# JoeyYoung/adapcc

Measured on AMD Instinct MI355X. Metric: gpt2_ddp_tokens_per_sec, higher is better.
Workload: dtype bf16; 1 GPU; model=gpt2-small-124M, global_batch=128, seq_len=1024, parallelism=dp1, bucket_cap_mb=100, hipgraph=True, precision=bf16, transport=native

## Files before the change

adapcc_amd/models/gpt2.py:

```python

from __future__ import annotations

import math
from dataclasses import dataclass

import torch
import torch.nn as nn
import torch.nn.functional as F

from ..ops.fused import FusedLayerNorm


@dataclass
class GPT2Config:
    vocab_size: int = 50257
    n_positions: int = 1024
    n_embd: int = 768
    n_layer: int = 12
    n_head: int = 12
    dropout: float = 0.0
    resid_dropout: float = 0.0
    n_kv_head: int = None

    @classmethod
    def small(cls) -> "GPT2Config":
        return cls()

    @classmethod
    def tiny(cls) -> "GPT2Config":
        return cls(vocab_size=2048, n_positions=256, n_embd=128, n_layer=2,
                   n_head=4)

    @classmethod
    def medium(cls) -> "GPT2Config":
        return cls(n_embd=1024, n_layer=24, n_head=16)


class CausalSelfAttention(nn.Module):
    def __init__(self, cfg: GPT2Config):
        super().__init__()
        assert cfg.n_embd % cfg.n_head == 0
        self.n_head = cfg.n_head
        self.n_kv_head = (cfg.n_head if cfg.n_kv_head is None
                          else cfg.n_kv_head)
        assert self.n_kv_head >= 1 and cfg.n_head % self.n_kv_head == 0
        head_dim = cfg.n_embd // cfg.n_head
        self.c_attn = nn.Linear(
            cfg.n_embd, (cfg.n_head + 2 * self.n_kv_head) * head_dim)
        self.c_proj = nn.Linear(cfg.n_embd, cfg.n_embd)
        self.dropout = cfg.dropout

    def forward(self, x: torch.Tensor,
                cu_seqlens: torch.Tensor = None) -> torch.Tensor:
        from ..ops import attention

        p = self.dropout if self.training else 0.0
        if cu_seqlens is not None:
            qkv = self.c_attn(x)
            y = attention.flash_attention_qkv_varlen(
                qkv.view(qkv.shape[1], qkv.shape[2]), self.n_head,
                cu_seqlens, dropout_p=p, n_kv_head=self.n_kv_head)
            return self.c_proj(y.view(1, y.shape[0], y.shape[1]))
        return self.c_proj(attention.flash_attention_qkv(
            self.c_attn(x), self.n_head,
            dropout_p=self.dropout if self.training else 0.0,
            n_kv_head=self.n_kv_head,
        ))


class MLP(nn.Module):
    def __init__(self, cfg: GPT2Config):
        super().__init__()
        self.c_fc = nn.Linear(cfg.n_embd, 4 * cfg.n_embd)
        self.c_proj = nn.Linear(4 * cfg.n_embd, cfg.n_embd)

    def forward(self, x: torch.Tensor) -> torch.Tensor:
        from ..ops.fused import fused_gelu

        return self.c_proj(fused_gelu(self.c_fc(x)))


class Block(nn.Module):
    def __init__(self, cfg: GPT2Config):
        super().__init__()
        self.ln_1 = FusedLayerNorm(cfg.n_embd)
        self.attn = CausalSelfAttention(cfg)
        self.ln_2 = FusedLayerNorm(cfg.n_embd)
        self.mlp = MLP(cfg)

    def forward(self, x: torch.Tensor,
                cu_seqlens: torch.Tensor = None) -> torch.Tensor:
        if cu_seqlens is None:
            x = x + self.attn(self.ln_1(x))
        else:
            x = x + self.attn(self.ln_1(x), cu_seqlens)
        x = x + self.mlp(self.ln_2(x))
        return x

    def forward_resid_dropout(self, x: torch.Tensor, y: torch.Tensor,
                              next_ln: nn.LayerNorm, p: float, site: int,
                              cu_seqlens: torch.Tensor = None):
        from ..ops.fused import fused_dropout_add_layer_norm

        a = self.attn(y) if cu_seqlens is None else self.attn(y, cu_seqlens)
        x, y = fused_dropout_add_layer_norm(
            a, x, self.ln_2.weight, self.ln_2.bias, self.ln_2.eps,
            dropout_p=p, site=site)
        return fused_dropout_add_layer_norm(
            self.mlp(y), x, next_ln.weight, next_ln.bias, next_ln.eps,
            dropout_p=p, site=site + 1)


class GPT2(nn.Module):
    def __init__(self, cfg: GPT2Config):
        super().__init__()
        self.cfg = cfg
        self.wte = nn.Embedding(cfg.vocab_size, cfg.n_embd)
        self.wpe = nn.Embedding(cfg.n_positions, cfg.n_embd)
        self.drop = nn.Dropout(cfg.dropout)
        self.h = nn.ModuleList(Block(cfg) for _ in range(cfg.n_layer))
        self.ln_f = FusedLayerNorm(cfg.n_embd)
        self.lm_head = nn.Linear(cfg.n_embd, cfg.vocab_size, bias=False)
        self.lm_head.weight = self.wte.weight
        self.apply(self._init)
        for name, p in self.named_parameters():
            if name.endswith("c_proj.weight"):
                nn.init.normal_(p, mean=0.0,
                                std=0.02 / math.sqrt(2 * cfg.n_layer))

    @staticmethod
    def _init(m: nn.Module) -> None:
        if isinstance(m, nn.Linear):
            nn.init.normal_(m.weight, mean=0.0, std=0.02)
            if m.bias is not None:
                nn.init.zeros_(m.bias)
        elif isinstance(m, nn.Embedding):
            nn.init.normal_(m.weight, mean=0.0, std=0.02)

    def num_params(self, non_embedding: bool = True) -> int:
        n = sum(p.numel() for p in self.parameters())
        if non_embedding:
            n -= self.wpe.weight.numel()
        return n

    def _packed_positions(self, cu_seqlens: torch.Tensor,
                          total: int) -> torch.Tensor:
        rows = torch.arange(total, dtype=torch.int32,
                            device=cu_seqlens.device)
        ends = cu_seqlens[1:].contiguous()
        doc = torch.bucketize(rows, ends, right=True)
        doc = doc.clamp_(max=ends.numel() - 1)
        pos = rows - cu_seqlens[:-1][doc]
        return pos.clamp_(0, self.cfg.n_positions - 1).long()

    def forward(self, idx: torch.Tensor, targets: torch.Tensor = None,
                cu_seqlens: torch.Tensor = None):
        B, T = idx.shape
        if cu_seqlens is None:
            pos = torch.arange(T, device=idx.device)
            kw = {}
        else:
            if B != 1:
                raise ValueError("GPT2.forward: with cu_seqlens idx must be "
                                 f"[1, total], got {tuple(idx.shape)}")
            pos = self._packed_positions(cu_seqlens, T)
            kw = {"cu_seqlens": cu_seqlens}
        x = self.drop(self.wte(idx) + self.wpe(pos))
        if self.training and self.cfg.resid_dropout > 0.0:
            lns = [b.ln_1 for b in self.h[1:]] + [self.ln_f]
            y = self.h[0].ln_1(x)
            for i, block in enumerate(self.h):
                x, y = block.forward_resid_dropout(
                    x, y, lns[i], self.cfg.resid_dropout, site=2 * i, **kw)
            x = y
        else:
            for block in self.h:
                x = block(x, **kw)
            x = self.ln_f(x)
        logits = self.lm_head(x)
        loss = None
        if targets is not None:
            from ..ops.fused import fused_cross_entropy

            loss = fused_cross_entropy(
                logits.view(-1, logits.size(-1)), targets.view(-1)
            )
        return logits, loss
```

adapcc_amd/ops/build.py:

```python

from __future__ import annotations

import hashlib
import os
import subprocess
import sys
import sysconfig

PKG_DIR = os.path.dirname(os.path.dirname(os.path.abspath(__file__)))
CSRC = os.path.join(PKG_DIR, "ops", "csrc")
SOURCES = ["kernels.hip", "engine.hip", "plan.cpp", "lnorm.hip", "ce.hip",
           "attn.hip", "attn_probe.hip", "gelu.hip", "moe.hip",
           "bindings.hip"]
HEADERS = ["common.h", "engine.h", "plan.h", "attn_frag.h", "attn_drop.h"]
OUT_SO = os.path.join(PKG_DIR, "_core.so")
STAMP = os.path.join(PKG_DIR, "ops", ".build_stamp")

HIPCC = os.environ.get("ADAPCC_HIPCC", "/opt/rocm/bin/hipcc")
ARCH = os.environ.get("PYTORCH_ROCM_ARCH", "gfx950")


def _source_hash() -> str:
    h = hashlib.sha256()
    for name in SOURCES + HEADERS:
        with open(os.path.join(CSRC, name), "rb") as f:
            h.update(f.read())
    h.update(ARCH.encode())
    return h.hexdigest()


def needs_build() -> bool:
    if not os.path.exists(OUT_SO):
        return True
    if not os.path.exists(STAMP):
        return True
    with open(STAMP) as f:
        return f.read().strip() != _source_hash()


def build(verbose: bool = True, force: bool = False) -> str:
    if not force and not needs_build():
        return OUT_SO
    import pybind11

    py_inc = sysconfig.get_paths()["include"]
    cmd = [
        HIPCC,
        f"--offload-arch={ARCH}",
        "-O3",
        "-std=c++17",
        "-fPIC",
        "-shared",
        "-fvisibility=hidden",
        f"-I{CSRC}",
        f"-I{pybind11.get_include()}",
        f"-I{py_inc}",
    ]
    cmd += [os.path.join(CSRC, s) for s in SOURCES]
    cmd += ["-o", OUT_SO]
    if verbose:
        print("[adapcc_amd.build]", " ".join(cmd), file=sys.stderr)
    subprocess.run(cmd, check=True)
    with open(STAMP, "w") as f:
        f.write(_source_hash())
    return OUT_SO


if __name__ == "__main__":
    build(force="--force" in sys.argv)
```

adapcc_amd/ops/csrc/attn.hip:

```cpp

#include <algorithm>
#include <cmath>
#include <cstdint>
#include <stdexcept>
#include <string>
#include <type_traits>

#include "attn_drop.h"
#include "attn_frag.h"

namespace adapcc {

namespace {

constexpr int kQT = 128;
constexpr float kNegBig = -3.0e38f;
constexpr float kLog2e = 1.4426950408889634f;
constexpr float kLn2 = 0.6931471805599453f;

struct TStride {
  long sb, sh, ss;
};

template <typename T>
__device__ __forceinline__ T* plane(T* x, const TStride& s, int b, int h) {
  return x + (long)b * s.sb + (long)h * s.sh;
}

struct FaParams {
  const __bf16 *q, *k, *v;
  __bf16* o;
  float* lse;
  TStride qs, ks, vs, os;
  int H, S;
  float scale;
  const __bf16* dout;
  float* delta;
  __bf16 *dq, *dk, *dv;
  TStride dos_, dqs, dks, dvs;
  const long* seed;
  unsigned drop_thr;
  float drop_rp;
  const int4* tmap;
  int total;
  int G;
};

struct VarlenTile {
  int seq, tile, start, len;
};

__device__ __forceinline__ VarlenTile varlen_tile(const FaParams& p) {
  const int4 e = p.tmap[blockIdx.x];
  return {e.x, e.y, e.z, e.w};
}

template <bool kVarlen, typename T>
__device__ __forceinline__ T* seq_plane(T* x, const TStride& s, int b, int h,
                                        long row0) {
  if constexpr (kVarlen)
    return x + (long)h * s.sh + row0 * s.ss;
  else
    return plane(x, s, b, h);
}

template <bool kGqa>
__device__ __forceinline__ int kv_head(int h, int G) {
  if constexpr (kGqa)
    return h / G;
  else
    return h;
}

__device__ __forceinline__ bool varlen_idle(const VarlenTile& t) {
  return t.seq < 0 || (long)t.tile * kQT >= t.len;
}

template <bool kRagged>
__device__ __forceinline__ long ld_row(long row, int S) {
  return kRagged ? (long)min((int)row, S - 1) : row;
}
template <bool kRagged>
__device__ __forceinline__ int ld_row32(int row, int S) {
  return kRagged ? min(row, S - 1) : row;
}

template <bool kCausal, bool kRagged>
__device__ __forceinline__ int tile_count(int qt, int S) {
  if (kCausal && kRagged) return min((qt + 1) * (kQT / 64), (S + 63) / 64);
  return kCausal ? (qt + 1) * (kQT / 64) : (S + 63) / 64;
}

template <bool kCausal, bool kRagged>
__device__ __forceinline__ bool key_masked(int kglob, int qrow, int qlim,
                                           int S) {
  if (kCausal && kRagged) return kglob > qlim;
  return kCausal ? kglob > qrow : kglob >= S;
}

constexpr int kHalfImg = 4096;
constexpr int kImg = 2 * kHalfImg;

template <int kHD>
constexpr int kTileImg = (kHD / 64) * kImg;

template <int kHD>
__device__ __forceinline__ char* img(char* base, int buf) {
  return base + buf * kTileImg<kHD>;
}

template <int kHD>
__device__ __forceinline__ bf16x8 read_row_chunk(const char* im, int lane,
                                                 int c) {
  if constexpr (kHD == 64)
    return read_row_frag(im, lane, c);
  else
    return read_row_frag(im + (c >> 2) * kImg, lane, c & 3);
}

template <int kHD>
__device__ __forceinline__ bf16x8 read_tr_blk(const char* im, int lane,
                                              int kb, int db) {
  if constexpr (kHD == 64)
    return read_tr_frag(im, lane, kb, db);
  else
    return read_tr_frag(im + (db >> 1) * kImg, lane, kb, db & 1);
}

struct RowPair {
  uint4 a, b;
};

__device__ __forceinline__ RowPair ld_pair(const __bf16* g, long ss, long r0,
                                           long r1, int scol) {
  return {*reinterpret_cast<const uint4*>(g + r0 * ss + scol),
          *reinterpret_cast<const uint4*>(g + r1 * ss + scol)};
}

__device__ __forceinline__ void st_pair(char* im, int srow, int scol,
                                        const RowPair& x) {
  *reinterpret_cast<uint4*>(im + row_img_byte(srow, scol)) = x.a;
  *reinterpret_cast<uint4*>(im + kHalfImg + row_img_byte(srow, scol)) = x.b;
}

template <int kHD>
struct RowTile {
  RowPair blk[kHD / 64];
};

template <int kHD>
__device__ __forceinline__ RowTile<kHD> ld_tile(const __bf16* g, long ss,
                                                long r0, long r1, int scol) {
  RowTile<kHD> x;
  x.blk[0] = ld_pair(g, ss, r0, r1, scol);
  if constexpr (kHD == 128) x.blk[1] = ld_pair(g + 64, ss, r0, r1, scol);
  return x;
}

template <int kHD>
__device__ __forceinline__ void st_tile(char* im, int srow, int scol,
                                        const RowTile<kHD>& x) {
  st_pair(im, srow, scol, x.blk[0]);
  if constexpr (kHD == 128) st_pair(im + kImg, srow, scol, x.blk[1]);
}

constexpr int kSideDelta = 128;

struct SideVal {
  float lse2, delta;
};

__device__ __forceinline__ SideVal ld_side(const float* lseg,
                                           const float* deltag, int row) {
  return {lseg[row] * kLog2e, deltag[row]};
}

__device__ __forceinline__ float* side_buf(float* side, int buf) {
  return side + (buf ? 64 : 0);
}

__device__ __forceinline__ void st_side(float* side, int buf, unsigned i,
                                        const SideVal& x) {
  side[(buf ? 64 : 0) + i] = x.lse2;
  (side + kSideDelta)[(buf ? 64 : 0) + i] = x.delta;
}

template <bool kDrop>
constexpr int kPartBytes = kDrop ? 2 * 64 * 4 : 0;

__device__ __forceinline__ unsigned* part_buf(unsigned* part, int buf) {
  return part + (buf ? 64 : 0);
}

__device__ __forceinline__ void store4_bf16(__bf16* dst, float a, float b,
                                            float c, float d) {
  unsigned lo, hi;
  asm("v_cvt_pk_bf16_f32 %0, %2, %3\n\t"
      "v_cvt_pk_bf16_f32 %1, %4, %5"
      : "=&v"(lo), "=&v"(hi)
      : "v"(a), "v"(b), "v"(c), "v"(d));
  uint2 st = {lo, hi};
  *reinterpret_cast<uint2*>(dst) = st;
}

__device__ __forceinline__ float p_elem(float s, float c1, float off) {
  return __builtin_amdgcn_exp2f(__builtin_fmaf(s, c1, -off));
}

__device__ __forceinline__ float ds_elem(float pe, float dp, float delta,
                                         float scale) {
  return pe * (dp - delta) * scale;
}

template <int kHD, bool kCausal, bool kRagged, bool kDrop,
          bool kVarlen = false, bool kGqa = false>
__global__ __launch_bounds__(256, kHD == 64 ? 3 : 2) void fa_fwd_kernel(
    FaParams p) {
  static_assert(kHD == 64 || kHD == 128, "head_dim 64 or 128");
  static_assert(kVarlen ? kRagged : !(kCausal && kRagged),
                "fixed-length causal needs S % 128 == 0; varlen is ragged");
  constexpr int kNC = kHD / 16;
  constexpr int kNB = kHD / 32;
  __shared__ __attribute__((aligned(16))) char
      smem[4 * kTileImg<kHD> + kPartBytes<kDrop>];
  char* const kimg = smem;
  char* const vimg = smem + 2 * kTileImg<kHD>;
  [[maybe_unused]] unsigned* const kpart =
      reinterpret_cast<unsigned*>(smem + 4 * kTileImg<kHD>);

  const int lane = threadIdx.x & 63;
  const int wave = threadIdx.x >> 6;
  const int hi = lane >> 5;
  int qt = blockIdx.x, bh = blockIdx.y, b, h, S = p.S;
  long row0 = 0;
  if constexpr (kVarlen) {
    const VarlenTile vt = varlen_tile(p);
    if (varlen_idle(vt)) return;
    qt = vt.tile;
    b = 0;
    h = blockIdx.y;
    bh = vt.seq * p.H + h;
    S = vt.len;
    row0 = vt.start;
  } else {
    b = bh / p.H;
    h = bh % p.H;
  }

  const __bf16* qg = seq_plane<kVarlen>(p.q, p.qs, b, h, row0);
  const int hk = kv_head<kGqa>(h, p.G);
  const __bf16* kg = seq_plane<kVarlen>(p.k, p.ks, b, hk, row0);
  const __bf16* vg = seq_plane<kVarlen>(p.v, p.vs, b, hk, row0);
  __bf16* og = seq_plane<kVarlen>(p.o, p.os, b, h, row0);
  float* lseg =
      p.lse + (kVarlen ? (long)h * p.total + row0 : (long)bh * S);

  const int qb = qt * kQT + wave * 32;
  const int qrow = qb + (lane & 31);
  const long qld = ld_row<kRagged>((long)qrow, S);
  [[maybe_unused]] const int qlim = min(qrow, S - 1);

  bf16x8 qf[kNC];
#pragma unroll
  for (int c = 0; c < kNC; ++c)
    qf[c] = *reinterpret_cast<const bf16x8*>(
        qg + qld * p.qs.ss + c * 16 + hi * 8);

  f32x16 acc0 = {}, acc1 = {};
  [[maybe_unused]] f32x16 acc2 = {}, acc3 = {};
  float m = kNegBig, ssum = 0.f;
  const float c1 = p.scale * kLog2e;
  float mc = m * c1;
  const float thr = 8.0f / p.scale;

  const int srow = threadIdx.x >> 3;
  const int scol = (threadIdx.x & 7) * 8;
  const int n64 = tile_count<kCausal, kRagged>(qt, S);

  [[maybe_unused]] unsigned dqa = 0, seed_hi = 0;
  if constexpr (kDrop) {
    const unsigned long sd = (unsigned long)*p.seed;
    dqa = drop_q_part((unsigned)sd, bh, qrow);
    seed_hi = (unsigned)(sd >> 32);
  }

  {
    const long r0 = ld_row<kRagged>((long)srow, S);
    const long r1 = ld_row<kRagged>((long)(srow + 32), S);
    st_tile<kHD>(img<kHD>(kimg, 0), srow, scol,
                 ld_tile<kHD>(kg, p.ks.ss, r0, r1, scol));
    st_tile<kHD>(img<kHD>(vimg, 0), srow, scol,
                 ld_tile<kHD>(vg, p.vs.ss, r0, r1, scol));
    if constexpr (kDrop)
      if (threadIdx.x < 64)
        kpart[threadIdx.x] = drop_k_part(seed_hi, bh, threadIdx.x);
  }
  __syncthreads();

  int cur = 0;
  for (int t = 0; t < n64; ++t) {
    RowTile<kHD> nk, nv;
    const bool pref = t + 1 < n64;
    if (pref) {
      const long kb = (long)(t + 1) * 64 + srow;
      const long kb0 = ld_row<kRagged>(kb, S);
      const long kb1 = ld_row<kRagged>(kb + 32, S);
      nk = ld_tile<kHD>(kg, p.ks.ss, kb0, kb1, scol);
      nv = ld_tile<kHD>(vg, p.vs.ss, kb0, kb1, scol);
      if constexpr (kDrop)
        if (threadIdx.x < 64)
          part_buf(kpart, cur ^ 1)[threadIdx.x] =
              drop_k_part(seed_hi, bh, (t + 1) * 64 + threadIdx.x);
    }

#pragma unroll
    for (int half = 0; half < 2; ++half) {
      const int kbase = t * 64 + half * 32;
      if (kCausal) {
        if (kbase > qb + 31) break;
      }
      if (kRagged) {
        if (kbase >= S || qb >= S) break;
      }
      const char* ki = img<kHD>(kimg, cur) + half * kHalfImg;
      const char* vi = img<kHD>(vimg, cur) + half * kHalfImg;

      f32x16 s = {};
      __builtin_amdgcn_s_setprio(1);
#pragma unroll
      for (int c = 0; c < kNC; ++c)
        s = mfma(read_row_chunk<kHD>(ki, lane, c), qf[c], s);
      __builtin_amdgcn_s_setprio(0);

      float pv[16];
      float tmax = kNegBig;
      if ((kCausal && kbase + 31 > qb) || (kRagged && kbase + 31 >= S)) {
#pragma unroll
        for (int r = 0; r < 16; ++r) {
          const int kglob = kbase + crow(r, hi);
          pv[r] = key_masked<kCausal, kRagged>(kglob, qrow, qlim, S)
                      ? kNegBig
                      : s[r];
          tmax = fmaxf(tmax, pv[r]);
        }
      } else {
#pragma unroll
        for (int r = 0; r < 16; ++r) {
          pv[r] = s[r];
          tmax = fmaxf(tmax, pv[r]);
        }
      }
      tmax = fmaxf(tmax, __shfl_xor(tmax, 32, 64));
      if (!__all(tmax <= m + thr)) {
        const float mnew = fmaxf(m, tmax);
        const float alpha = __builtin_amdgcn_exp2f((m - mnew) * c1);
        m = mnew;
        mc = m * c1;
        ssum *= alpha;
#pragma unroll
        for (int r = 0; r < 16; ++r) {
          acc0[r] *= alpha;
          acc1[r] *= alpha;
          if constexpr (kNB == 4) {
            acc2[r] *= alpha;
            acc3[r] *= alpha;
          }
        }
      }

      float psum = 0.f;
#pragma unroll
      for (int r = 0; r < 16; ++r) {
        pv[r] = p_elem(pv[r], c1, mc);
        psum += pv[r];
      }
      ssum += psum;

      if constexpr (kDrop) {
        const unsigned* kp = part_buf(kpart, cur) + half * 32;
#pragma unroll
        for (int r = 0; r < 16; ++r)
          if (!drop_keep_parts(dqa, kp[crow(r, hi)], p.drop_thr))
            pv[r] = 0.f;
      }

      const bf16x8 p0 = pack_frag(&pv[0]);
      const bf16x8 p1 = pack_frag(&pv[8]);

      __builtin_amdgcn_s_setprio(1);
      acc0 = mfma(read_tr_blk<kHD>(vi, lane, 0, 0), p0, acc0);
      acc0 = mfma(read_tr_blk<kHD>(vi, lane, 1, 0), p1, acc0);
      acc1 = mfma(read_tr_blk<kHD>(vi, lane, 0, 1), p0, acc1);
      acc1 = mfma(read_tr_blk<kHD>(vi, lane, 1, 1), p1, acc1);
      if constexpr (kNB == 4) {
        acc2 = mfma(read_tr_blk<kHD>(vi, lane, 0, 2), p0, acc2);
        acc2 = mfma(read_tr_blk<kHD>(vi, lane, 1, 2), p1, acc2);
        acc3 = mfma(read_tr_blk<kHD>(vi, lane, 0, 3), p0, acc3);
        acc3 = mfma(read_tr_blk<kHD>(vi, lane, 1, 3), p1, acc3);
      }
      __builtin_amdgcn_s_setprio(0);
    }

    if (pref) {
      st_tile<kHD>(img<kHD>(kimg, cur ^ 1), srow, scol, nk);
      st_tile<kHD>(img<kHD>(vimg, cur ^ 1), srow, scol, nv);
    }
    __syncthreads();
    cur ^= 1;
  }

  const float stot = ssum + __shfl_xor(ssum, 32, 64);
  float inv = 1.f / stot;
  if constexpr (kDrop) inv = p.drop_rp / stot;
  if (kRagged && qrow >= S) return;
  if ((lane >> 5) == 0)
    lseg[qrow] = p.scale * m + __builtin_amdgcn_logf(stot) * kLn2;

  __bf16* orow = og + (long)qrow * p.os.ss;
#pragma unroll
  for (int db = 0; db < kNB; ++db) {
    const f32x16& a = db == 3 ? acc3 : db == 2 ? acc2 : db ? acc1 : acc0;
#pragma unroll
    for (int mq = 0; mq < 4; ++mq)
      store4_bf16(orow + db * 32 + 8 * mq + 4 * hi, a[4 * mq] * inv,
                  a[4 * mq + 1] * inv, a[4 * mq + 2] * inv,
                  a[4 * mq + 3] * inv);
  }
}

__device__ __forceinline__ float dot8_tree(bf16x8 a, bf16x8 b) {
  union {
    bf16x8 f;
    unsigned u[4];
  } x, y;
  x.f = a;
  y.f = b;
  float pr[4];
#pragma unroll
  for (int i = 0; i < 4; ++i) {
    const float ev = __builtin_fmaf(__uint_as_float(x.u[i] << 16),
                                    __uint_as_float(y.u[i] << 16), 0.f);
    pr[i] = __builtin_fmaf(__uint_as_float(x.u[i] & 0xffff0000u),
                           __uint_as_float(y.u[i] & 0xffff0000u), ev);
  }
  return (pr[0] + pr[1]) + (pr[2] + pr[3]);
}

template <int kHD, bool kCausal, bool kRagged, bool kDrop,
          bool kVarlen = false, bool kGqa = false>
__global__ __launch_bounds__(256, kHD == 64 ? 3 : 2) void fa_bwd_dq_kernel(
    FaParams p) {
  static_assert(kHD == 64 || kHD == 128, "head_dim 64 or 128");
  static_assert(kVarlen ? kRagged : !(kCausal && kRagged),
                "fixed-length causal needs S % 128 == 0; varlen is ragged");
  constexpr int kNC = kHD / 16;
  constexpr int kNB = kHD / 32;
  __shared__ __attribute__((aligned(16))) char
      smem[4 * kTileImg<kHD> + kPartBytes<kDrop>];
  char* const kimg = smem;
  char* const vimg = smem + 2 * kTileImg<kHD>;
  [[maybe_unused]] unsigned* const kpart =
      reinterpret_cast<unsigned*>(smem + 4 * kTileImg<kHD>);

  const int lane = threadIdx.x & 63;
  const int wave = threadIdx.x >> 6;
  const int hi = lane >> 5;
  int qt = blockIdx.x, bh = blockIdx.y, b, h, S = p.S;
  long row0 = 0;
  if constexpr (kVarlen) {
    const VarlenTile vt = varlen_tile(p);
    if (varlen_idle(vt)) return;
    qt = vt.tile;
    b = 0;
    h = blockIdx.y;
    bh = vt.seq * p.H + h;
    S = vt.len;
    row0 = vt.start;
  } else {
    b = bh / p.H;
    h = bh % p.H;
  }

  const __bf16* qg = seq_plane<kVarlen>(p.q, p.qs, b, h, row0);
  const int hk = kv_head<kGqa>(h, p.G);
  const __bf16* kg = seq_plane<kVarlen>(p.k, p.ks, b, hk, row0);
  const __bf16* vg = seq_plane<kVarlen>(p.v, p.vs, b, hk, row0);
  const __bf16* dog = seq_plane<kVarlen>(p.dout, p.dos_, b, h, row0);
  const __bf16* og = seq_plane<kVarlen>(p.o, p.os, b, h, row0);
  __bf16* dqg = seq_plane<kVarlen>(p.dq, p.dqs, b, h, row0);
  const long lrow0 = kVarlen ? (long)h * p.total + row0 : (long)bh * S;

  const int qb = qt * kQT + wave * 32;
  const int qrow = qb + (lane & 31);
  const long qld = ld_row32<kRagged>(qrow, S);
  [[maybe_unused]] const int qlim = min(qrow, S - 1);

  bf16x8 qf[kNC], dof[kNC];
  float n16[kNC];
#pragma unroll
  for (int c = 0; c < kNC; ++c) {
    dof[c] = *reinterpret_cast<const bf16x8*>(
        dog + qld * p.dos_.ss + c * 16 + hi * 8);
    const float n8 = dot8_tree(
        dof[c], *reinterpret_cast<const bf16x8*>(
                    og + qld * p.os.ss + c * 16 + hi * 8));
    n16[c] = n8 + __shfl_xor(n8, 32, 64);
  }
#pragma unroll
  for (int c = 0; c < kNC; ++c)
    qf[c] = *reinterpret_cast<const bf16x8*>(
        qg + qld * p.qs.ss + c * 16 + hi * 8);
  const float lse2 = p.lse[lrow0 + qld] * kLog2e;
  float dvq = (n16[0] + n16[1]) + (n16[2] + n16[3]);
  if constexpr (kHD == 128)
    dvq = dvq + ((n16[4] + n16[5]) + (n16[6] + n16[7]));
  if (hi == 0 && (!kRagged || qrow < S))
    p.delta[lrow0 + qrow] = dvq;
  const float c1 = p.scale * kLog2e;

  f32x16 dacc0 = {}, dacc1 = {};
  [[maybe_unused]] f32x16 dacc2 = {}, dacc3 = {};

  const int srow = threadIdx.x >> 3;
  const int scol = (threadIdx.x & 7) * 8;
  const int n64 = tile_count<kCausal, kRagged>(qt, S);

  [[maybe_unused]] unsigned dqa = 0, seed_hi = 0;
  if constexpr (kDrop) {
    const unsigned long sd = (unsigned long)*p.seed;
    dqa = drop_q_part((unsigned)sd, bh, qrow);
    seed_hi = (unsigned)(sd >> 32);
  }
  {
    const long r0 = ld_row32<kRagged>(srow, S);
    const long r1 = ld_row32<kRagged>(srow + 32, S);
    st_tile<kHD>(img<kHD>(kimg, 0), srow, scol,
                 ld_tile<kHD>(kg, p.ks.ss, r0, r1, scol));
    st_tile<kHD>(img<kHD>(vimg, 0), srow, scol,
                 ld_tile<kHD>(vg, p.vs.ss, r0, r1, scol));
    if constexpr (kDrop)
      if (threadIdx.x < 64)
        kpart[threadIdx.x] = drop_k_part(seed_hi, bh, threadIdx.x);
  }
  __syncthreads();

  int cur = 0;
  for (int t = 0; t < n64; ++t) {
    RowTile<kHD> nk, nv;
    const bool pref = t + 1 < n64;
    if (pref) {
      const long kb0 = ld_row32<kRagged>((t + 1) * 64 + srow, S);
      const long kb1 = ld_row32<kRagged>((t + 1) * 64 + srow + 32, S);
      nk = ld_tile<kHD>(kg, p.ks.ss, kb0, kb1, scol);
      nv = ld_tile<kHD>(vg, p.vs.ss, kb0, kb1, scol);
      if constexpr (kDrop)
        if (threadIdx.x < 64)
          part_buf(kpart, cur ^ 1)[threadIdx.x] =
              drop_k_part(seed_hi, bh, (t + 1) * 64 + threadIdx.x);
    }

#pragma unroll
    for (int half = 0; half < 2; ++half) {
      const int kbase = t * 64 + half * 32;
      if (kCausal) {
        if (kbase > qb + 31) break;
      }
      if (kRagged) {
        if (kbase >= S || qb >= S) break;
      }
      const char* ki = img<kHD>(kimg, cur) + half * kHalfImg;
      const char* vi = img<kHD>(vimg, cur) + half * kHalfImg;

      f32x16 s = {}, dp = {};
      __builtin_amdgcn_s_setprio(1);
#pragma unroll
      for (int c = 0; c < kNC; ++c) {
        s = mfma(read_row_chunk<kHD>(ki, lane, c), qf[c], s);
        dp = mfma(read_row_chunk<kHD>(vi, lane, c), dof[c], dp);
      }
      __builtin_amdgcn_s_setprio(0);

      float ds[16];
      [[maybe_unused]] const unsigned* kp =
          part_buf(kpart, cur) + half * 32;
      auto dpk = [&](int r) {
        if constexpr (kDrop)
          return drop_keep_parts(dqa, kp[crow(r, hi)], p.drop_thr)
                     ? dp[r] * p.drop_rp
                     : 0.f;
        else
          return dp[r];
      };
      if (kDrop) {
        const int lim = kCausal ? (kRagged ? qlim : qrow)
                        : kRagged ? S - 1
                                  : 0x7fffffff;
#pragma unroll
        for (int r = 0; r < 16; ++r) {
          const int kglob = kbase + crow(r, hi);
          const float pe = kglob > lim ? 0.f : p_elem(s[r], c1, lse2);
          ds[r] = ds_elem(pe, dpk(r), dvq, p.scale);
        }
      } else if ((kCausal && kbase + 31 > qb) ||
                 (kRagged && kbase + 31 >= S)) {
#pragma unroll
        for (int r = 0; r < 16; ++r) {
          const int kglob = kbase + crow(r, hi);
          const float pe = key_masked<kCausal, kRagged>(kglob, qrow, qlim, S)
                               ? 0.f
                               : p_elem(s[r], c1, lse2);
          ds[r] = ds_elem(pe, dpk(r), dvq, p.scale);
        }
      } else {
#pragma unroll
        for (int r = 0; r < 16; ++r)
          ds[r] = ds_elem(p_elem(s[r], c1, lse2), dpk(r), dvq, p.scale);
      }
      const bf16x8 d0 = pack_frag(&ds[0]);
      const bf16x8 d1 = pack_frag(&ds[8]);
      __builtin_amdgcn_s_setprio(1);
      dacc0 = mfma(read_tr_blk<kHD>(ki, lane, 0, 0), d0, dacc0);
      dacc0 = mfma(read_tr_blk<kHD>(ki, lane, 1, 0), d1, dacc0);
      dacc1 = mfma(read_tr_blk<kHD>(ki, lane, 0, 1), d0, dacc1);
      dacc1 = mfma(read_tr_blk<kHD>(ki, lane, 1, 1), d1, dacc1);
      if constexpr (kNB == 4) {
        dacc2 = mfma(read_tr_blk<kHD>(ki, lane, 0, 2), d0, dacc2);
        dacc2 = mfma(read_tr_blk<kHD>(ki, lane, 1, 2), d1, dacc2);
        dacc3 = mfma(read_tr_blk<kHD>(ki, lane, 0, 3), d0, dacc3);
        dacc3 = mfma(read_tr_blk<kHD>(ki, lane, 1, 3), d1, dacc3);
      }
      __builtin_amdgcn_s_setprio(0);
    }

    if (pref) {
      st_tile<kHD>(img<kHD>(kimg, cur ^ 1), srow, scol, nk);
      st_tile<kHD>(img<kHD>(vimg, cur ^ 1), srow, scol, nv);
    }
    __syncthreads();
    cur ^= 1;
  }

  if (kRagged && qrow >= S) return;
  __bf16* drow = dqg + (long)qrow * p.dqs.ss;
#pragma unroll
  for (int db = 0; db < kNB; ++db) {
    const f32x16& a = db == 3 ? dacc3 : db == 2 ? dacc2 : db ? dacc1 : dacc0;
#pragma unroll
    for (int mq = 0; mq < 4; ++mq)
      store4_bf16(drow + db * 32 + 8 * mq + 4 * hi, a[4 * mq], a[4 * mq + 1],
                  a[4 * mq + 2], a[4 * mq + 3]);
  }
}

template <int kHD, bool kCausal, bool kRagged, bool kDrop,
          bool kVarlen = false, bool kGqa = false>
__global__ __launch_bounds__(256, kHD == 64 ? 2 : 1) void fa_bwd_dkv_kernel(
    FaParams p) {
  static_assert(kHD == 64 || kHD == 128, "head_dim 64 or 128");
  static_assert(kVarlen ? kRagged : !(kCausal && kRagged),
                "fixed-length causal needs S % 128 == 0; varlen is ragged");
  constexpr int kNC = kHD / 16;
  constexpr int kNB = kHD / 32;
  __shared__ __attribute__((aligned(16))) char
      smem[4 * kTileImg<kHD> + 1024 + kPartBytes<kDrop>];
  char* const qimg = smem;
  char* const doimg = smem + 2 * kTileImg<kHD>;
  float* const side =
      reinterpret_cast<float*>(smem + 4 * kTileImg<kHD>);
  [[maybe_unused]] unsigned* const qpart =
      reinterpret_cast<unsigned*>(smem + 4 * kTileImg<kHD> + 1024);

  const int lane = threadIdx.x & 63;
  const int wave = threadIdx.x >> 6;
  const int hi = lane >> 5;
  int kt = blockIdx.x, bh = blockIdx.y, b, h, S = p.S;
  int hk;
  long row0 = 0;
  if constexpr (kVarlen) {
    const VarlenTile vt = varlen_tile(p);
    if (varlen_idle(vt)) return;
    kt = vt.tile;
    b = 0;
    hk = blockIdx.y;
    h = kGqa ? hk * p.G : hk;
    bh = vt.seq * p.H + h;
    S = vt.len;
    row0 = vt.start;
  } else if constexpr (kGqa) {
    const int Hk = p.H / p.G;
    b = bh / Hk;
    hk = bh % Hk;
    h = hk * p.G;
    bh = b * p.H + h;
  } else {
    b = bh / p.H;
    h = bh % p.H;
    hk = h;
  }

  const __bf16* qg = seq_plane<kVarlen>(p.q, p.qs, b, h, row0);
  const __bf16* kg = seq_plane<kVarlen>(p.k, p.ks, b, hk, row0);
  const __bf16* vg = seq_plane<kVarlen>(p.v, p.vs, b, hk, row0);
  const __bf16* dog = seq_plane<kVarlen>(p.dout, p.dos_, b, h, row0);
  __bf16* dkg = seq_plane<kVarlen>(p.dk, p.dks, b, hk, row0);
  __bf16* dvg = seq_plane<kVarlen>(p.dv, p.dvs, b, hk, row0);
  const long lrow0 = kVarlen ? (long)h * p.total + row0 : (long)bh * S;
  const float* lseg = p.lse + lrow0;
  const float* deltag = p.delta + lrow0;

  const int kbb = kt * kQT + wave * 32;
  const int krow = kbb + (lane & 31);
  const long kld = ld_row32<kRagged>(krow, S);

  bf16x8 kf[kNC], vf[kNC];
#pragma unroll
  for (int c = 0; c < kNC; ++c) {
    kf[c] = *reinterpret_cast<const bf16x8*>(
        kg + kld * p.ks.ss + c * 16 + hi * 8);
    vf[c] = *reinterpret_cast<const bf16x8*>(
        vg + kld * p.vs.ss + c * 16 + hi * 8);
  }

  const float c1 = p.scale * kLog2e;
  f32x16 dvacc0 = {}, dvacc1 = {}, dkacc0 = {}, dkacc1 = {};
  [[maybe_unused]] f32x16 dvacc2 = {}, dvacc3 = {}, dkacc2 = {}, dkacc3 = {};

  const int srow = threadIdx.x >> 3;
  const int scol = (threadIdx.x & 7) * 8;
  const int t0 = kCausal ? (kVarlen ? kt * (kQT / 64) : kt) : 0;
  const int n64 = (S + 63) / 64;

  [[maybe_unused]] unsigned dkb = 0, seed_lo = 0;
  [[maybe_unused]] unsigned seed_hi = 0;
  [[maybe_unused]] int bhc = bh;
  if constexpr (kDrop) {
    const unsigned long sd = (unsigned long)*p.seed;
    seed_lo = (unsigned)sd;
    dkb = drop_k_part((unsigned)(sd >> 32), bh, krow);
    if constexpr (kGqa) seed_hi = (unsigned)(sd >> 32);
  }
  [[maybe_unused]] int stage_left = 0, walk_left = 0;
  if constexpr (kGqa) stage_left = walk_left = p.G - 1;

  {
    const int qb0 = t0 * 64;
    const long r0 = ld_row32<kRagged>(qb0 + srow, S);
    const long r1 = ld_row32<kRagged>(qb0 + srow + 32, S);
    st_tile<kHD>(img<kHD>(qimg, 0), srow, scol,
                 ld_tile<kHD>(qg, p.qs.ss, r0, r1, scol));
    st_tile<kHD>(img<kHD>(doimg, 0), srow, scol,
                 ld_tile<kHD>(dog, p.dos_.ss, r0, r1, scol));
    if (threadIdx.x < 64) {
      const int rq = ld_row32<kRagged>(qb0 + (int)threadIdx.x, S);
      st_side(side, 0, threadIdx.x, ld_side(lseg, deltag, rq));
      if constexpr (kDrop)
        qpart[threadIdx.x] = drop_q_part(seed_lo, bh, qb0 + threadIdx.x);
    }
  }
  __syncthreads();

  int cur = 0;
  for (int t = t0; t < n64; ++t) {
    RowTile<kHD> nq, nd;
    SideVal ns = {0.f, 0.f};
    bool pref = t + 1 < n64;
    int tn = t + 1;
    if constexpr (kGqa) {
      if (!pref && stage_left > 0) {
        --stage_left;
        pref = true;
        tn = t0;
        qg += p.qs.sh;
        dog += p.dos_.sh;
        lseg += kVarlen ? p.total : S;
        deltag += kVarlen ? p.total : S;
        ++bh;
      }
    }
    if (pref) {
      const int qb1 = tn * 64;
      const long r0 = ld_row32<kRagged>(qb1 + srow, S);
      const long r1 = ld_row32<kRagged>(qb1 + srow + 32, S);
      nq = ld_tile<kHD>(qg, p.qs.ss, r0, r1, scol);
      nd = ld_tile<kHD>(dog, p.dos_.ss, r0, r1, scol);
      if (threadIdx.x < 64) {
        const int rq = ld_row32<kRagged>(qb1 + (int)threadIdx.x, S);
        ns = ld_side(lseg, deltag, rq);
        if constexpr (kDrop)
          part_buf(qpart, cur ^ 1)[threadIdx.x] =
              drop_q_part(seed_lo, bh, qb1 + threadIdx.x);
      }
    }

#pragma unroll
    for (int half = 0; half < 2; ++half) {
      const int qbase = t * 64 + half * 32;
      if (kCausal) {
        if (qbase + 31 < kbb) continue;
      }
      if (kRagged) {
        if (qbase >= S || kbb >= S) break;
      }
      const char* qi = img<kHD>(qimg, cur) + half * kHalfImg;
      const char* di = img<kHD>(doimg, cur) + half * kHalfImg;
      const float* lsec = side_buf(side, cur) + half * 32;
      const float* dc = lsec + kSideDelta;

      f32x16 sacc = {}, dp = {};
      __builtin_amdgcn_s_setprio(1);
#pragma unroll
      for (int c = 0; c < kNC; ++c) {
        sacc = mfma(read_row_chunk<kHD>(qi, lane, c), kf[c], sacc);
        dp = mfma(read_row_chunk<kHD>(di, lane, c), vf[c], dp);
      }
      __builtin_amdgcn_s_setprio(0);

      float pv[16], ds[16];
      [[maybe_unused]] bool keep[16];
      if constexpr (kDrop) {
        const unsigned* qp = part_buf(qpart, cur) + half * 32;
#pragma unroll
        for (int r = 0; r < 16; ++r) {
          keep[r] = drop_keep_parts(qp[crow(r, hi)], dkb, p.drop_thr);
          dp[r] = keep[r] ? dp[r] * p.drop_rp : 0.f;
        }
      }
      if ((kCausal && qbase < kbb + 31) || (kRagged && qbase + 31 >= S)) {
#pragma unroll
        for (int r = 0; r < 16; ++r) {
          const int qglob = qbase + crow(r, hi);
          pv[r] = ((kCausal && qglob < krow) || (kRagged && qglob >= S))
                      ? 0.f
                      : p_elem(sacc[r], c1, lsec[crow(r, hi)]);
          ds[r] = ds_elem(pv[r], dp[r], dc[crow(r, hi)], p.scale);
        }
      } else {
#pragma unroll
        for (int r = 0; r < 16; ++r) {
          pv[r] = p_elem(sacc[r], c1, lsec[crow(r, hi)]);
          ds[r] = ds_elem(pv[r], dp[r], dc[crow(r, hi)], p.scale);
        }
      }
      if constexpr (kDrop) {
#pragma unroll
        for (int r = 0; r < 16; ++r)
          if (!keep[r]) pv[r] = 0.f;
      }
      const bf16x8 p0 = pack_frag(&pv[0]);
      const bf16x8 p1 = pack_frag(&pv[8]);
      __builtin_amdgcn_s_setprio(1);
      dvacc0 = mfma(p0, read_tr_blk<kHD>(di, lane, 0, 0), dvacc0);
      dvacc0 = mfma(p1, read_tr_blk<kHD>(di, lane, 1, 0), dvacc0);
      dvacc1 = mfma(p0, read_tr_blk<kHD>(di, lane, 0, 1), dvacc1);
      dvacc1 = mfma(p1, read_tr_blk<kHD>(di, lane, 1, 1), dvacc1);
      if constexpr (kNB == 4) {
        dvacc2 = mfma(p0, read_tr_blk<kHD>(di, lane, 0, 2), dvacc2);
        dvacc2 = mfma(p1, read_tr_blk<kHD>(di, lane, 1, 2), dvacc2);
        dvacc3 = mfma(p0, read_tr_blk<kHD>(di, lane, 0, 3), dvacc3);
        dvacc3 = mfma(p1, read_tr_blk<kHD>(di, lane, 1, 3), dvacc3);
      }
      __builtin_amdgcn_s_setprio(0);
      const bf16x8 e0 = pack_frag(&ds[0]);
      const bf16x8 e1 = pack_frag(&ds[8]);
      __builtin_amdgcn_s_setprio(1);
      dkacc0 = mfma(e0, read_tr_blk<kHD>(qi, lane, 0, 0), dkacc0);
      dkacc0 = mfma(e1, read_tr_blk<kHD>(qi, lane, 1, 0), dkacc0);
      dkacc1 = mfma(e0, read_tr_blk<kHD>(qi, lane, 0, 1), dkacc1);
      dkacc1 = mfma(e1, read_tr_blk<kHD>(qi, lane, 1, 1), dkacc1);
      if constexpr (kNB == 4) {
        dkacc2 = mfma(e0, read_tr_blk<kHD>(qi, lane, 0, 2), dkacc2);
        dkacc2 = mfma(e1, read_tr_blk<kHD>(qi, lane, 1, 2), dkacc2);
        dkacc3 = mfma(e0, read_tr_blk<kHD>(qi, lane, 0, 3), dkacc3);
        dkacc3 = mfma(e1, read_tr_blk<kHD>(qi, lane, 1, 3), dkacc3);
      }
      __builtin_amdgcn_s_setprio(0);
    }

    if (pref) {
      st_tile<kHD>(img<kHD>(qimg, cur ^ 1), srow, scol, nq);
      st_tile<kHD>(img<kHD>(doimg, cur ^ 1), srow, scol, nd);
      if (threadIdx.x < 64) st_side(side, cur ^ 1, threadIdx.x, ns);
    }
    __syncthreads();
    cur ^= 1;
    if constexpr (kGqa) {
      if (t + 1 == n64 && walk_left > 0) {
        --walk_left;
        t = t0 - 1;
        if constexpr (kDrop) dkb = drop_k_part(seed_hi, ++bhc, krow);
      }
    }
  }

  __syncthreads();
  float* scratch = reinterpret_cast<float*>(smem) + wave * (32 * kHD);
#pragma unroll
  for (int t = 0; t < 2; ++t) {
    const f32x16& a0 = t ? dkacc0 : dvacc0;
    const f32x16& a1 = t ? dkacc1 : dvacc1;
    [[maybe_unused]] const f32x16& a2 = t ? dkacc2 : dvacc2;
    [[maybe_unused]] const f32x16& a3 = t ? dkacc3 : dvacc3;
    if (kDrop && t == 0) {
#pragma unroll
      for (int r = 0; r < 16; ++r) {
        scratch[crow(r, hi) * kHD + (lane & 31)] = a0[r] * p.drop_rp;
        scratch[crow(r, hi) * kHD + 32 + (lane & 31)] = a1[r] * p.drop_rp;
        if constexpr (kNB == 4) {
          scratch[crow(r, hi) * kHD + 64 + (lane & 31)] = a2[r] * p.drop_rp;
          scratch[crow(r, hi) * kHD + 96 + (lane & 31)] = a3[r] * p.drop_rp;
        }
      }
    } else {
#pragma unroll
      for (int r = 0; r < 16; ++r) {
        scratch[crow(r, hi) * kHD + (lane & 31)] = a0[r];
        scratch[crow(r, hi) * kHD + 32 + (lane & 31)] = a1[r];
        if constexpr (kNB == 4) {
          scratch[crow(r, hi) * kHD + 64 + (lane & 31)] = a2[r];
          scratch[crow(r, hi) * kHD + 96 + (lane & 31)] = a3[r];
        }
      }
    }
    __builtin_amdgcn_s_waitcnt(0);
    __bf16* outg = (t ? dkg : dvg);
    const TStride& os = t ? p.dks : p.dvs;
    const int row = lane >> 1;
    const int dhalf = (lane & 1) * (kHD / 2);
#pragma unroll
    for (int mq = 0; mq < kHD / 8; ++mq) {
      const float* src = scratch + row * kHD + dhalf + mq * 4;
      if (!kRagged || kbb + row < S)
        store4_bf16(outg + (long)(kbb + row) * os.ss + dhalf + mq * 4, src[0],
                    src[1], src[2], src[3]);
    }
    __syncthreads();
  }
}

__global__ __launch_bounds__(256) void fa_dropout_mask_kernel(
    uint8_t* out, const long* seed, int S, unsigned thr) {
  const long n = (long)S * S;
  const long i = (long)blockIdx.x * 256 + threadIdx.x;
  if (i >= n) return;
  const unsigned bh = blockIdx.y;
  out[bh * n + i] =
      drop_keep(*seed, bh, (unsigned)(i / S), (unsigned)(i % S), thr);
}

constexpr int kIntMin = -2147483647 - 1;

template <bool kMax>
__device__ __forceinline__ int plan_scan(int* buf, int x, int* all) {
  const int t = threadIdx.x;
  constexpr int kId = kMax ? kIntMin : 0;
  buf[t] = x;
  __syncthreads();
  for (int d = 1; d < 256; d <<= 1) {
    const int y = t >= d ? buf[t - d] : kId;
    __syncthreads();
    buf[t] = kMax ? max(buf[t], y) : buf[t] + y;
    __syncthreads();
  }
  const int excl = t ? buf[t - 1] : kId;
  *all = buf[255];
  __syncthreads();
  return excl;
}

__device__ __forceinline__ int clamp_row(int x, int total) {
  return min(max(x, 0), total);
}

__global__ __launch_bounds__(256) void fa_varlen_plan_kernel(
    const int* cu, int n_seqs, int total, int max_tiles, int4* tmap) {
  __shared__ int buf[256];
  const int t = threadIdx.x;
  const int per = (n_seqs + 255) / 256;
  const int i0 = min(t * per, n_seqs), i1 = min(i0 + per, n_seqs);

  int mx = kIntMin;
  for (int i = i0; i < i1; ++i) mx = max(mx, cu[i + 1]);
  int unused;
  const int m0 = max(cu[0], plan_scan<true>(buf, mx, &unused));

  int tiles = 0;
  for (int i = i0, m = m0; i < i1; ++i) {
    const int e = clamp_row(m, total);
    m = max(m, cu[i + 1]);
    tiles += (clamp_row(m, total) - e + kQT - 1) / kQT;
  }
  int n_tiles;
  int at = plan_scan<false>(buf, tiles, &n_tiles);

  for (int i = i0, m = m0; i < i1; ++i) {
    const int e = clamp_row(m, total);
    m = max(m, cu[i + 1]);
    const int len = clamp_row(m, total) - e;
    for (int j = 0; j * kQT < len; ++j, ++at)
      if (at < max_tiles) tmap[at] = make_int4(i, j, e, len);
  }
  for (int x = n_tiles + t; x < max_tiles; x += 256)
    tmap[x] = make_int4(-1, -1, -1, -1);
}

TStride stride_at(const long* s, int i) {
  return {s[3 * i], s[3 * i + 1], s[3 * i + 2]};
}

unsigned drop_threshold(double p) {
  const double t = std::nearbyint(p * 4294967296.0);
  return (unsigned)std::min(std::max(t, 1.0), 4294967295.0);
}

void check_drop(const char* name, double p, const long* seed) {
  if (!(p >= 0.0 && p < 1.0))
    throw std::runtime_error(std::string(name) + ": need 0 <= dropout_p < 1");
  if (p > 0.0 && seed == nullptr)
    throw std::runtime_error(std::string(name) +
                             ": dropout needs a device seed");
}

void set_drop(FaParams& p, double dropout_p, const long* seed) {
  p.seed = seed;
  p.drop_thr = drop_threshold(dropout_p);
  p.drop_rp = (float)(1.0 / (1.0 - dropout_p));
}

void check_len(const char* name, int S, bool causal) {
  if (S < 1) throw std::runtime_error(std::string(name) + ": S < 1");
  if (causal && S % kQT != 0)
    throw std::runtime_error(std::string(name) +
                             ": causal needs S % 128 == 0");
}

void check_varlen(const char* name, int total, int n_seqs, int H) {
  if (total < 1) throw std::runtime_error(std::string(name) + ": total < 1");
  if (n_seqs < 1)
    throw std::runtime_error(std::string(name) + ": n_seqs < 1");
  if (H < 1) throw std::runtime_error(std::string(name) + ": H < 1");
  if ((long)total / kQT + n_seqs > 0x7fffffffL - kQT || total > 0x7fffff00)
    throw std::runtime_error(std::string(name) + ": too many tiles");
}

int varlen_max_tiles(int total, int n_seqs) { return total / kQT + n_seqs; }

template <typename F>
void with_mode(bool causal, int S, bool drop, bool varlen, F&& f) {
  auto g = [&](auto d) {
    if (varlen) {
      if (causal)
        f(std::true_type{}, std::true_type{}, d, std::true_type{});
      else
        f(std::false_type{}, std::true_type{}, d, std::true_type{});
    } else if (causal) {
      f(std::true_type{}, std::false_type{}, d, std::false_type{});
    } else if (S % kQT == 0) {
      f(std::false_type{}, std::false_type{}, d, std::false_type{});
    } else {
      f(std::false_type{}, std::true_type{}, d, std::false_type{});
    }
  };
  if (drop)
    g(std::true_type{});
  else
    g(std::false_type{});
}

FaParams fwd_params(const char* name, const void* q, const void* k,
                    const void* v, void* o, float* lse, int H, int n_kv_head,
                    int S, const long* strides, float scale) {
  const int Hk = n_kv_head == 0 ? H : n_kv_head;
  if (H < 1 || Hk < 1 || H % Hk != 0)
    throw std::runtime_error(std::string(name) + ": need n_kv_head >= 1 that "
                             "divides H, got H " + std::to_string(H) +
                             ", n_kv_head " + std::to_string(n_kv_head));
  FaParams p = {};
  p.G = H / Hk;
  p.q = (const __bf16*)q;
  p.k = (const __bf16*)k;
  p.v = (const __bf16*)v;
  p.o = (__bf16*)o;
  p.lse = lse;
  p.qs = stride_at(strides, 0);
  p.ks = stride_at(strides, 1);
  p.vs = stride_at(strides, 2);
  p.os = stride_at(strides, 3);
  p.H = H;
  p.S = S;
  p.scale = scale;
  return p;
}

void bwd_params(FaParams& p, const void* do_, float* delta, void* dq,
                void* dk, void* dv, const long* strides) {
  p.dout = (const __bf16*)do_;
  p.delta = delta;
  p.dq = (__bf16*)dq;
  p.dk = (__bf16*)dk;
  p.dv = (__bf16*)dv;
  p.dos_ = stride_at(strides, 4);
  p.dqs = stride_at(strides, 5);
  p.dks = stride_at(strides, 6);
  p.dvs = stride_at(strides, 7);
}

void set_varlen(FaParams& p, const int* tmap, int total) {
  if (tmap == nullptr) throw std::runtime_error("fa_varlen: no tile map");
  p.tmap = reinterpret_cast<const int4*>(tmap);
  p.total = total;
}

template <typename F>
void with_head_dim(const char* name, int head_dim, F&& f) {
  if (head_dim == 64)
    f(std::integral_constant<int, 64>{});
  else if (head_dim == 128)
    f(std::integral_constant<int, 128>{});
  else
    throw std::runtime_error(std::string(name) +
                             ": head_dim must be 64 or 128, got " +
                             std::to_string(head_dim));
}

template <typename F>
void with_gqa(int G, F&& f) {
  if (G > 1)
    f(std::true_type{});
  else
    f(std::false_type{});
}

void launch_fwd(const FaParams& p, dim3 grid, int head_dim, bool causal,
                bool drop, bool varlen, hipStream_t stream) {
  with_head_dim("fa_forward", head_dim, [&](auto hd) {
    with_mode(causal, p.S, drop, varlen, [&](auto c, auto r, auto d, auto vl) {
      with_gqa(p.G, [&](auto gq) {
        constexpr int kHD = decltype(hd)::value;
        constexpr bool kC = decltype(c)::value, kR = decltype(r)::value,
                       kD = decltype(d)::value, kV = decltype(vl)::value,
                       kG = decltype(gq)::value;
        hipLaunchKernelGGL((fa_fwd_kernel<kHD, kC, kR, kD, kV, kG>), grid,
                           dim3(256), 0, stream, p);
      });
    });
  });
}

void launch_bwd(const FaParams& p, dim3 grid, int head_dim, bool causal,
                bool drop, bool varlen, hipStream_t stream) {
  const dim3 kv_grid(grid.x, grid.y / p.G);
  with_head_dim("fa_backward", head_dim, [&](auto hd) {
    with_mode(causal, p.S, drop, varlen, [&](auto c, auto r, auto d, auto vl) {
      with_gqa(p.G, [&](auto gq) {
        constexpr int kHD = decltype(hd)::value;
        constexpr bool kC = decltype(c)::value, kR = decltype(r)::value,
                       kD = decltype(d)::value, kV = decltype(vl)::value,
                       kG = decltype(gq)::value;
        hipLaunchKernelGGL((fa_bwd_dq_kernel<kHD, kC, kR, kD, kV, kG>), grid,
                           dim3(256), 0, stream, p);
        hipLaunchKernelGGL((fa_bwd_dkv_kernel<kHD, kC, kR, kD, kV, kG>),
                           kv_grid, dim3(256), 0, stream, p);
      });
    });
  });
}

}

unsigned fa_drop_threshold(double p) { return drop_threshold(p); }

void fa_forward(const void* q, const void* k, const void* v, void* o,
                float* lse, int B, int H, int S, const long* strides,
                float scale, hipStream_t stream, bool causal,
                double dropout_p, const long* seed, int head_dim,
                int n_kv_head) {
  check_len("fa_forward", S, causal);
  check_drop("fa_forward", dropout_p, seed);
  FaParams p = fwd_params("fa_forward", q, k, v, o, lse, H, n_kv_head, S,
                          strides, scale);
  set_drop(p, dropout_p, seed);
  const dim3 grid((S + kQT - 1) / kQT, B * H);
  launch_fwd(p, grid, head_dim, causal, dropout_p > 0.0, false, stream);
}

void fa_backward(const void* q, const void* k, const void* v, const void* o,
                 const void* do_, const float* lse, float* delta, void* dq,
                 void* dk, void* dv, int B, int H, int S, const long* strides,
                 float scale, hipStream_t stream, bool causal,
                 double dropout_p, const long* seed, int head_dim,
                 int n_kv_head) {
  check_len("fa_backward", S, causal);
  check_drop("fa_backward", dropout_p, seed);
  FaParams p = fwd_params("fa_backward", q, k, v, const_cast<void*>(o),
                          const_cast<float*>(lse), H, n_kv_head, S, strides,
                          scale);
  set_drop(p, dropout_p, seed);
  bwd_params(p, do_, delta, dq, dk, dv, strides);
  const dim3 grid((S + kQT - 1) / kQT, B * H);
  launch_bwd(p, grid, head_dim, causal, dropout_p > 0.0, false, stream);
}

void fa_varlen_plan(const int* cu_seqlens, int n_seqs, int total, int* tmap,
                    hipStream_t stream) {
  check_varlen("fa_varlen_plan", total, n_seqs, 1);
  if (cu_seqlens == nullptr || tmap == nullptr)
    throw std::runtime_error("fa_varlen_plan: null pointer");
  hipLaunchKernelGGL(fa_varlen_plan_kernel, dim3(1), dim3(256), 0, stream,
                     cu_seqlens, n_seqs, total,
                     varlen_max_tiles(total, n_seqs),
                     reinterpret_cast<int4*>(tmap));
}

void fa_varlen_forward(const void* q, const void* k, const void* v, void* o,
                       float* lse, const int* tmap, int total, int n_seqs,
                       int H, const long* strides, float scale,
                       hipStream_t stream, bool causal, double dropout_p,
                       const long* seed, int head_dim, int n_kv_head) {
  check_varlen("fa_varlen_forward", total, n_seqs, H);
  check_drop("fa_varlen_forward", dropout_p, seed);
  FaParams p = fwd_params("fa_varlen_forward", q, k, v, o, lse, H, n_kv_head,
                          0, strides, scale);
  set_drop(p, dropout_p, seed);
  set_varlen(p, tmap, total);
  const dim3 grid(varlen_max_tiles(total, n_seqs), H);
  launch_fwd(p, grid, head_dim, causal, dropout_p > 0.0, true, stream);
}

void fa_varlen_backward(const void* q, const void* k, const void* v,
                        const void* o, const void* do_, const float* lse,
                        float* delta, void* dq, void* dk, void* dv,
                        const int* tmap, int total, int n_seqs, int H,
                        const long* strides, float scale, hipStream_t stream,
                        bool causal, double dropout_p, const long* seed,
                        int head_dim, int n_kv_head) {
  check_varlen("fa_varlen_backward", total, n_seqs, H);
  check_drop("fa_varlen_backward", dropout_p, seed);
  FaParams p = fwd_params("fa_varlen_backward", q, k, v,
                          const_cast<void*>(o), const_cast<float*>(lse), H,
                          n_kv_head, 0, strides, scale);
  set_drop(p, dropout_p, seed);
  set_varlen(p, tmap, total);
  bwd_params(p, do_, delta, dq, dk, dv, strides);
  const dim3 grid(varlen_max_tiles(total, n_seqs), H);
  launch_bwd(p, grid, head_dim, causal, dropout_p > 0.0, true, stream);
}

void fa_dropout_mask(uint8_t* out, const long* seed, int B, int H, int S,
                     double dropout_p, hipStream_t stream) {
  if (S < 1 || B < 1 || H < 1)
    throw std::runtime_error("fa_dropout_mask: empty shape");
  if (seed == nullptr)
    throw std::runtime_error("fa_dropout_mask: needs a device seed");
  check_drop("fa_dropout_mask", dropout_p, seed);
  const long n = (long)S * S;
  const dim3 grid((unsigned)((n + 255) / 256), B * H);
  hipLaunchKernelGGL(fa_dropout_mask_kernel, grid, dim3(256), 0, stream, out,
                     seed, S, drop_threshold(dropout_p));
}

}
```

adapcc_amd/ops/csrc/bindings.hip:

```cpp

#include <pybind11/pybind11.h>
#include <pybind11/stl.h>

#include "common.h"
#include "engine.h"
#include "plan.h"

namespace py = pybind11;
using adapcc::Engine;

static py::dict plan_to_dict(const adapcc::PlanData& p) {
  py::list cs, rs, bs;
  for (const auto& u : p.cunits) {
    py::dict d;
    d["tree"] = u.tree; d["chunk"] = u.chunk;
    d["offset"] = u.offset_elems; d["count"] = u.count_elems;
    d["flag_space"] = (int)u.flag_space;
    py::list nl;
    for (int i = 0; i < u.nnotify; ++i) nl.append(u.notify_rank[i]);
    d["notify_to"] = nl;
    cs.append(d);
  }
  for (const auto& u : p.runits) {
    py::dict d;
    d["tree"] = u.tree; d["chunk"] = u.chunk;
    d["offset"] = u.offset_elems; d["count"] = u.count_elems;
    py::list srcs;
    for (int s = 0; s < u.nsrc; ++s)
      srcs.append(py::make_tuple(u.src_rank[s], (int)u.src_kind[s]));
    d["srcs"] = srcs;
    d["include_self"] = (bool)u.include_self;
    d["notify"] = (bool)u.notify_parent; d["consumer"] = u.parent_rank;
    d["is_root"] = (bool)u.is_root;
    py::list kids;
    for (int c = 0; c < u.nchildren; ++c) kids.append(u.child_rank[c]);
    d["publish_to"] = kids;
    rs.append(d);
  }
  for (const auto& u : p.bunits) {
    py::dict d;
    d["tree"] = u.tree; d["chunk"] = u.chunk;
    d["src_offset"] = u.src_offset_elems; d["dst_offset"] = u.dst_offset_elems;
    d["count"] = u.count_elems;
    d["parent"] = u.parent_rank; d["parent_kind"] = (int)u.parent_kind;
    d["forward"] = (bool)u.forward;
    py::list kids;
    for (int c = 0; c < u.nchildren; ++c) kids.append(u.child_rank[c]);
    d["publish_to"] = kids;
    bs.append(d);
  }
  py::dict out;
  out["copy"] = cs;
  out["reduce"] = rs;
  out["bcast"] = bs;
  out["chunk_elems"] = p.chunk_elems;
  return out;
}

namespace adapcc {
void launch_local_reduce(Dtype dt, void* dst, const void* const* srcs_dev,
                         int nsrc, long count, RedOp op, float scale,
                         hipStream_t stream);
bool ln_supported_api(long cols, int dtype);
void ln_forward(int dtype, const void* x, const void* w, const void* b,
                void* y, float* mean, float* rstd, long rows, long cols,
                float eps, hipStream_t stream);
void ln_backward(int dtype, const void* dy, const void* x, const void* w,
                 const float* mean, const float* rstd, void* dx,
                 float* ws_gamma, float* ws_beta, long rows, long cols,
                 int nblocks, hipStream_t stream);
void ln_dropadd_forward(int dtype, const void* h, const void* res,
                        const void* w, const void* b, void* x_new, void* y,
                        float* mean, float* rstd, long rows, long cols,
                        float eps, double dropout_p, const long* seed,
                        unsigned site, hipStream_t stream);
void ln_dropadd_backward(int dtype, const void* dy, const void* dx_new,
                         const void* x_new, const void* w, const float* mean,
                         const float* rstd, void* dres, void* dh,
                         float* ws_gamma, float* ws_beta, long rows,
                         long cols, int nblocks, double dropout_p,
                         const long* seed, unsigned site,
                         hipStream_t stream);
void ce_forward(int dtype, const void* logits, const void* targets,
                float* loss, float* lse, long rows, long cols,
                long ignore_index, hipStream_t stream);
void ce_backward(int dtype, const void* logits, const void* targets,
                 const float* lse, const float* gscale, void* dlogits,
                 long rows, long cols, long ignore_index, hipStream_t stream);
void fa_forward(const void* q, const void* k, const void* v, void* o,
                float* lse, int B, int H, int S, const long* strides,
                float scale, hipStream_t stream, bool causal,
                double dropout_p, const long* seed, int head_dim,
                int n_kv_head);
void fa_backward(const void* q, const void* k, const void* v, const void* o,
                 const void* do_, const float* lse, float* delta, void* dq,
                 void* dk, void* dv, int B, int H, int S, const long* strides,
                 float scale, hipStream_t stream, bool causal,
                 double dropout_p, const long* seed, int head_dim,
                 int n_kv_head);
void fa_dropout_mask(uint8_t* out, const long* seed, int B, int H, int S,
                     double dropout_p, hipStream_t stream);
void fa_varlen_plan(const int* cu_seqlens, int n_seqs, int total, int* tmap,
                    hipStream_t stream);
void fa_varlen_forward(const void* q, const void* k, const void* v, void* o,
                       float* lse, const int* tmap, int total, int n_seqs,
                       int H, const long* strides, float scale,
                       hipStream_t stream, bool causal, double dropout_p,
                       const long* seed, int head_dim, int n_kv_head);
void fa_varlen_backward(const void* q, const void* k, const void* v,
                        const void* o, const void* do_, const float* lse,
                        float* delta, void* dq, void* dk, void* dv,
                        const int* tmap, int total, int n_seqs, int H,
                        const long* strides, float scale, hipStream_t stream,
                        bool causal, double dropout_p, const long* seed,
                        int head_dim, int n_kv_head);
void mfma_probe(const void* a, const void* b, float* c, hipStream_t stream);
void gelu_forward(int dtype, const void* x, void* y, long n,
                  hipStream_t stream);
void gelu_backward(int dtype, const void* x, const void* dy, void* dx, long n,
                   hipStream_t stream);
void moe_route(int dtype, const void* logits, float* gate_p, int* expert,
               int* slot, int* src, int* counts, int* offs, int* totals,
               long ntok, long E, long cap, hipStream_t stream);
void moe_route_bwd(int dtype, const void* logits, const float* gate_p,
                   const int* expert, const int* slot, const float* dgate,
                   void* dlogits, long ntok, long E, hipStream_t stream);
void moe_route_topk(int dtype, const void* logits, int k, int normalize,
                    float* gate, float* pmax, int* expert, int* slot,
                    int* src, int* src_choice, int* load, float* aux,
                    int* counts, int* offs, int* totals, float* psum,
                    long ntok, long E, long cap, hipStream_t stream);
void moe_route_topk_bwd(int dtype, const void* logits, int k, int normalize,
                        const float* pmax, const float* gate,
                        const int* expert, const int* slot,
                        const float* dgate, const int* load,
                        const float* daux, void* dlogits, long ntok, long E,
                        hipStream_t stream);
void moe_gather(int dtype, const void* in, long in_rows, const int* map,
                const float* scale, int scale_by_src, const int* choice,
                int nchoice, void* out, long rows, long d,
                hipStream_t stream);
void moe_gather2(int dtype, const void* in, long in_rows, const int* map,
                 const float* scale, void* out, long rows, long d,
                 hipStream_t stream);
void moe_rowdot(int dtype, const void* a, const void* b, long b_rows,
                const int* map, float* out, long rows, long d, int a_shift,
                hipStream_t stream);
void tr_probe(float* out, int kb, int db, hipStream_t stream);
void pack_probe(float* out, hipStream_t stream);
}

PYBIND11_MODULE(_core, m) {
  m.doc() = "adapcc_amd native engine (MI355X / gfx950)";

  m.def("local_reduce",
        [](uintptr_t dst, const std::vector<uintptr_t>& srcs, long count,
           int dtype, int op, float scale, uintptr_t stream) {
          if (srcs.empty()) throw std::runtime_error("no sources");
          void** d_srcs = nullptr;
          hipError_t e = hipMalloc(&d_srcs, srcs.size() * sizeof(void*));
          if (e != hipSuccess) throw std::runtime_error(hipGetErrorString(e));
          e = hipMemcpy(d_srcs, srcs.data(), srcs.size() * sizeof(void*),
                        hipMemcpyHostToDevice);
          if (e != hipSuccess) throw std::runtime_error(hipGetErrorString(e));
          adapcc::launch_local_reduce(
              (adapcc::Dtype)dtype, reinterpret_cast<void*>(dst),
              (const void* const*)d_srcs, (int)srcs.size(), count,
              (adapcc::RedOp)op, scale, reinterpret_cast<hipStream_t>(stream));
          e = hipGetLastError();
          if (e != hipSuccess) throw std::runtime_error(hipGetErrorString(e));
          e = hipStreamSynchronize(reinterpret_cast<hipStream_t>(stream));
          (void)hipFree(d_srcs);
          if (e != hipSuccess) throw std::runtime_error(hipGetErrorString(e));
        },
        py::arg("dst"), py::arg("srcs"), py::arg("count"), py::arg("dtype"),
        py::arg("op"), py::arg("scale") = 1.0f, py::arg("stream") = 0);

  m.def("ln_supported", &adapcc::ln_supported_api, py::arg("cols"),
        py::arg("dtype"));
  m.def("ln_fwd",
        [](int dtype, uintptr_t x, uintptr_t w, uintptr_t b, uintptr_t y,
           uintptr_t mean, uintptr_t rstd, long rows, long cols, float eps,
           uintptr_t stream) {
          adapcc::ln_forward(dtype, (const void*)x, (const void*)w,
                             (const void*)b, (void*)y, (float*)mean,
                             (float*)rstd, rows, cols, eps,
                             reinterpret_cast<hipStream_t>(stream));
          hipError_t e = hipGetLastError();
          if (e != hipSuccess) throw std::runtime_error(hipGetErrorString(e));
        });
  m.def("ln_bwd",
        [](int dtype, uintptr_t dy, uintptr_t x, uintptr_t w, uintptr_t mean,
           uintptr_t rstd, uintptr_t dx, uintptr_t wsg, uintptr_t wsb,
           long rows, long cols, int nblocks, uintptr_t stream) {
          adapcc::ln_backward(dtype, (const void*)dy, (const void*)x,
                              (const void*)w, (const float*)mean,
                              (const float*)rstd, (void*)dx, (float*)wsg,
                              (float*)wsb, rows, cols, nblocks,
                              reinterpret_cast<hipStream_t>(stream));
          hipError_t e = hipGetLastError();
          if (e != hipSuccess) throw std::runtime_error(hipGetErrorString(e));
        });
  m.def("ln_dropadd_fwd",
        [](int dtype, uintptr_t h, uintptr_t res, uintptr_t w, uintptr_t b,
           uintptr_t x_new, uintptr_t y, uintptr_t mean, uintptr_t rstd,
           long rows, long cols, float eps, uintptr_t stream,
           double dropout_p, uintptr_t seed, unsigned site) {
          adapcc::ln_dropadd_forward(
              dtype, (const void*)h, (const void*)res, (const void*)w,
              (const void*)b, (void*)x_new, (void*)y, (float*)mean,
              (float*)rstd, rows, cols, eps, dropout_p, (const long*)seed,
              site, reinterpret_cast<hipStream_t>(stream));
          hipError_t e = hipGetLastError();
          if (e != hipSuccess) throw std::runtime_error(hipGetErrorString(e));
        },
        py::arg("dtype"), py::arg("h"), py::arg("res"), py::arg("w"),
        py::arg("b"), py::arg("x_new"), py::arg("y"), py::arg("mean"),
        py::arg("rstd"), py::arg("rows"), py::arg("cols"), py::arg("eps"),
        py::arg("stream"), py::arg("dropout_p") = 0.0, py::arg("seed") = 0,
        py::arg("site") = 0);
  m.def("ln_dropadd_bwd",
        [](int dtype, uintptr_t dy, uintptr_t dx_new, uintptr_t x_new,
           uintptr_t w, uintptr_t mean, uintptr_t rstd, uintptr_t dres,
           uintptr_t dh, uintptr_t wsg, uintptr_t wsb, long rows, long cols,
           int nblocks, uintptr_t stream, double dropout_p, uintptr_t seed,
           unsigned site) {
          adapcc::ln_dropadd_backward(
              dtype, (const void*)dy, (const void*)dx_new,
              (const void*)x_new, (const void*)w, (const float*)mean,
              (const float*)rstd, (void*)dres, (void*)dh, (float*)wsg,
              (float*)wsb, rows, cols, nblocks, dropout_p, (const long*)seed,
              site, reinterpret_cast<hipStream_t>(stream));
          hipError_t e = hipGetLastError();
          if (e != hipSuccess) throw std::runtime_error(hipGetErrorString(e));
        },
        py::arg("dtype"), py::arg("dy"), py::arg("dx_new"), py::arg("x_new"),
        py::arg("w"), py::arg("mean"), py::arg("rstd"), py::arg("dres"),
        py::arg("dh"), py::arg("wsg"), py::arg("wsb"), py::arg("rows"),
        py::arg("cols"), py::arg("nblocks"), py::arg("stream"),
        py::arg("dropout_p") = 0.0, py::arg("seed") = 0,
        py::arg("site") = 0);

  m.def("ce_fwd",
        [](int dtype, uintptr_t logits, uintptr_t targets, uintptr_t loss,
           uintptr_t lse, long rows, long cols, long ignore_index,
           uintptr_t stream) {
          adapcc::ce_forward(dtype, (const void*)logits,
                             (const void*)targets, (float*)loss, (float*)lse,
                             rows, cols, ignore_index,
                             reinterpret_cast<hipStream_t>(stream));
          hipError_t e = hipGetLastError();
          if (e != hipSuccess) throw std::runtime_error(hipGetErrorString(e));
        });
  m.def("ce_bwd",
        [](int dtype, uintptr_t logits, uintptr_t targets, uintptr_t lse,
           uintptr_t gscale, uintptr_t dlogits, long rows, long cols,
           long ignore_index, uintptr_t stream) {
          adapcc::ce_backward(dtype, (const void*)logits,
                              (const void*)targets, (const float*)lse,
                              (const float*)gscale, (void*)dlogits, rows,
                              cols, ignore_index,
                              reinterpret_cast<hipStream_t>(stream));
          hipError_t e = hipGetLastError();
          if (e != hipSuccess) throw std::runtime_error(hipGetErrorString(e));
        });

  m.def("fa_fwd",
        [](uintptr_t q, uintptr_t k, uintptr_t v, uintptr_t o, uintptr_t lse,
           int B, int H, int S, const std::vector<long>& strides, float scale,
           uintptr_t stream, bool causal, double dropout_p, uintptr_t seed,
           int head_dim, int n_kv_head) {
          if (strides.size() != 12)
            throw std::runtime_error("fa_fwd: need 12 strides");
          adapcc::fa_forward((const void*)q, (const void*)k, (const void*)v,
                             (void*)o, (float*)lse, B, H, S, strides.data(),
                             scale, reinterpret_cast<hipStream_t>(stream),
                             causal, dropout_p, (const long*)seed, head_dim,
                             n_kv_head);
          hipError_t e = hipGetLastError();
          if (e != hipSuccess) throw std::runtime_error(hipGetErrorString(e));
        },
        py::arg("q"), py::arg("k"), py::arg("v"), py::arg("o"),
        py::arg("lse"), py::arg("B"), py::arg("H"), py::arg("S"),
        py::arg("strides"), py::arg("scale"), py::arg("stream"),
        py::arg("causal") = true, py::arg("dropout_p") = 0.0,
        py::arg("seed") = 0, py::arg("head_dim") = 64,
        py::arg("n_kv_head") = 0);
  m.def("fa_bwd",
        [](uintptr_t q, uintptr_t k, uintptr_t v, uintptr_t o, uintptr_t dout,
           uintptr_t lse, uintptr_t delta, uintptr_t dq, uintptr_t dk,
           uintptr_t dv, int B, int H, int S, const std::vector<long>& strides,
           float scale, uintptr_t stream, bool causal, double dropout_p,
           uintptr_t seed, int head_dim, int n_kv_head) {
          if (strides.size() != 24)
            throw std::runtime_error("fa_bwd: need 24 strides");
          adapcc::fa_backward((const void*)q, (const void*)k, (const void*)v,
                              (const void*)o, (const void*)dout,
                              (const float*)lse, (float*)delta, (void*)dq,
                              (void*)dk, (void*)dv, B, H, S, strides.data(),
                              scale, reinterpret_cast<hipStream_t>(stream),
                              causal, dropout_p, (const long*)seed, head_dim,
                              n_kv_head);
          hipError_t e = hipGetLastError();
          if (e != hipSuccess) throw std::runtime_error(hipGetErrorString(e));
        },
        py::arg("q"), py::arg("k"), py::arg("v"), py::arg("o"),
        py::arg("dout"), py::arg("lse"), py::arg("delta"), py::arg("dq"),
        py::arg("dk"), py::arg("dv"), py::arg("B"), py::arg("H"),
        py::arg("S"), py::arg("strides"), py::arg("scale"),
        py::arg("stream"), py::arg("causal") = true,
        py::arg("dropout_p") = 0.0, py::arg("seed") = 0,
        py::arg("head_dim") = 64, py::arg("n_kv_head") = 0);
  m.def("fa_dropout_mask",
        [](uintptr_t out, uintptr_t seed, int B, int H, int S,
           double dropout_p, uintptr_t stream) {
          adapcc::fa_dropout_mask((uint8_t*)out, (const long*)seed, B, H, S,
                                  dropout_p,
                                  reinterpret_cast<hipStream_t>(stream));
          hipError_t e = hipGetLastError();
          if (e != hipSuccess) throw std::runtime_error(hipGetErrorString(e));
        },
        py::arg("out"), py::arg("seed"), py::arg("B"), py::arg("H"),
        py::arg("S"), py::arg("dropout_p"), py::arg("stream"));
  m.def("fa_varlen_plan",
        [](uintptr_t cu_seqlens, int n_seqs, int total, uintptr_t tmap,
           uintptr_t stream) {
          adapcc::fa_varlen_plan((const int*)cu_seqlens, n_seqs, total,
                                 (int*)tmap,
                                 reinterpret_cast<hipStream_t>(stream));
          hipError_t e = hipGetLastError();
          if (e != hipSuccess) throw std::runtime_error(hipGetErrorString(e));
        },
        py::arg("cu_seqlens"), py::arg("n_seqs"), py::arg("total"),
        py::arg("tmap"), py::arg("stream"));
  m.def("fa_varlen_fwd",
        [](uintptr_t q, uintptr_t k, uintptr_t v, uintptr_t o, uintptr_t lse,
           uintptr_t tmap, int total, int n_seqs, int H,
           const std::vector<long>& strides, float scale, uintptr_t stream,
           bool causal, double dropout_p, uintptr_t seed, int head_dim,
           int n_kv_head) {
          if (strides.size() != 12)
            throw std::runtime_error("fa_varlen_fwd: need 12 strides");
          adapcc::fa_varlen_forward(
              (const void*)q, (const void*)k, (const void*)v, (void*)o,
              (float*)lse, (const int*)tmap, total, n_seqs, H, strides.data(),
              scale, reinterpret_cast<hipStream_t>(stream), causal, dropout_p,
              (const long*)seed, head_dim, n_kv_head);
          hipError_t e = hipGetLastError();
          if (e != hipSuccess) throw std::runtime_error(hipGetErrorString(e));
        },
        py::arg("q"), py::arg("k"), py::arg("v"), py::arg("o"),
        py::arg("lse"), py::arg("tmap"), py::arg("total"), py::arg("n_seqs"),
        py::arg("H"), py::arg("strides"), py::arg("scale"), py::arg("stream"),
        py::arg("causal") = true, py::arg("dropout_p") = 0.0,
        py::arg("seed") = 0, py::arg("head_dim") = 64,
        py::arg("n_kv_head") = 0);
  m.def("fa_varlen_bwd",
        [](uintptr_t q, uintptr_t k, uintptr_t v, uintptr_t o, uintptr_t dout,
           uintptr_t lse, uintptr_t delta, uintptr_t dq, uintptr_t dk,
           uintptr_t dv, uintptr_t tmap, int total, int n_seqs, int H,
           const std::vector<long>& strides, float scale, uintptr_t stream,
           bool causal, double dropout_p, uintptr_t seed, int head_dim,
           int n_kv_head) {
          if (strides.size() != 24)
            throw std::runtime_error("fa_varlen_bwd: need 24 strides");
          adapcc::fa_varlen_backward(
              (const void*)q, (const void*)k, (const void*)v, (const void*)o,
              (const void*)dout, (const float*)lse, (float*)delta, (void*)dq,
              (void*)dk, (void*)dv, (const int*)tmap, total, n_seqs, H,
              strides.data(), scale, reinterpret_cast<hipStream_t>(stream),
              causal, dropout_p, (const long*)seed, head_dim, n_kv_head);
          hipError_t e = hipGetLastError();
          if (e != hipSuccess) throw std::runtime_error(hipGetErrorString(e));
        },
        py::arg("q"), py::arg("k"), py::arg("v"), py::arg("o"),
        py::arg("dout"), py::arg("lse"), py::arg("delta"), py::arg("dq"),
        py::arg("dk"), py::arg("dv"), py::arg("tmap"), py::arg("total"),
        py::arg("n_seqs"), py::arg("H"), py::arg("strides"),
        py::arg("scale"), py::arg("stream"), py::arg("causal") = true,
        py::arg("dropout_p") = 0.0, py::arg("seed") = 0,
        py::arg("head_dim") = 64, py::arg("n_kv_head") = 0);
  m.def("mfma_probe",
        [](uintptr_t a, uintptr_t b, uintptr_t c, uintptr_t stream) {
          adapcc::mfma_probe((const void*)a, (const void*)b, (float*)c,
                             reinterpret_cast<hipStream_t>(stream));
          hipError_t e = hipGetLastError();
          if (e != hipSuccess) throw std::runtime_error(hipGetErrorString(e));
        });

  m.def("gelu_fwd",
        [](int dtype, uintptr_t x, uintptr_t y, long n, uintptr_t stream) {
          adapcc::gelu_forward(dtype, (const void*)x, (void*)y, n,
                               reinterpret_cast<hipStream_t>(stream));
          hipError_t e = hipGetLastError();
          if (e != hipSuccess) throw std::runtime_error(hipGetErrorString(e));
        });
  m.def("gelu_bwd",
        [](int dtype, uintptr_t x, uintptr_t dy, uintptr_t dx, long n,
           uintptr_t stream) {
          adapcc::gelu_backward(dtype, (const void*)x, (const void*)dy,
                                (void*)dx, n,
                                reinterpret_cast<hipStream_t>(stream));
          hipError_t e = hipGetLastError();
          if (e != hipSuccess) throw std::runtime_error(hipGetErrorString(e));
        });

  m.def("moe_route",
        [](int dtype, uintptr_t logits, uintptr_t gate_p, uintptr_t expert,
           uintptr_t slot, uintptr_t src, uintptr_t counts, uintptr_t offs,
           uintptr_t totals, long ntok, long E, long cap, uintptr_t stream) {
          adapcc::moe_route(dtype, (const void*)logits, (float*)gate_p,
                            (int*)expert, (int*)slot, (int*)src, (int*)counts,
                            (int*)offs, (int*)totals, ntok, E, cap,
                            reinterpret_cast<hipStream_t>(stream));
          hipError_t e = hipGetLastError();
          if (e != hipSuccess) throw std::runtime_error(hipGetErrorString(e));
        });
  m.def("moe_route_bwd",
        [](int dtype, uintptr_t logits, uintptr_t gate_p, uintptr_t expert,
           uintptr_t slot, uintptr_t dgate, uintptr_t dlogits, long ntok,
           long E, uintptr_t stream) {
          adapcc::moe_route_bwd(dtype, (const void*)logits,
                                (const float*)gate_p, (const int*)expert,
                                (const int*)slot, (const float*)dgate,
                                (void*)dlogits, ntok, E,
                                reinterpret_cast<hipStream_t>(stream));
          hipError_t e = hipGetLastError();
          if (e != hipSuccess) throw std::runtime_error(hipGetErrorString(e));
        });
  m.def("moe_route_topk",
        [](int dtype, uintptr_t logits, int k, bool normalize, uintptr_t gate,
           uintptr_t pmax, uintptr_t expert, uintptr_t slot, uintptr_t src,
           uintptr_t src_choice, uintptr_t load, uintptr_t aux,
           uintptr_t counts, uintptr_t offs, uintptr_t totals, uintptr_t psum,
           long ntok, long E, long cap, uintptr_t stream) {
          adapcc::moe_route_topk(
              dtype, (const void*)logits, k, normalize ? 1 : 0, (float*)gate,
              (float*)pmax, (int*)expert, (int*)slot, (int*)src,
              (int*)src_choice, (int*)load, (float*)aux, (int*)counts,
              (int*)offs, (int*)totals, (float*)psum, ntok, E, cap,
              reinterpret_cast<hipStream_t>(stream));
          hipError_t e = hipGetLastError();
          if (e != hipSuccess) throw std::runtime_error(hipGetErrorString(e));
        });
  m.def("moe_route_topk_bwd",
        [](int dtype, uintptr_t logits, int k, bool normalize, uintptr_t pmax,
           uintptr_t gate, uintptr_t expert, uintptr_t slot, uintptr_t dgate,
           uintptr_t load, uintptr_t daux, uintptr_t dlogits, long ntok,
           long E, uintptr_t stream) {
          adapcc::moe_route_topk_bwd(
              dtype, (const void*)logits, k, normalize ? 1 : 0,
              (const float*)pmax, (const float*)gate, (const int*)expert,
              (const int*)slot, (const float*)dgate, (const int*)load,
              (const float*)daux, (void*)dlogits, ntok, E,
              reinterpret_cast<hipStream_t>(stream));
          hipError_t e = hipGetLastError();
          if (e != hipSuccess) throw std::runtime_error(hipGetErrorString(e));
        });
  m.def("moe_gather",
        [](int dtype, uintptr_t in, long in_rows, uintptr_t map,
           uintptr_t scale, bool scale_by_src, uintptr_t choice, int nchoice,
           uintptr_t out, long rows, long d, uintptr_t stream) {
          adapcc::moe_gather(dtype, (const void*)in, in_rows, (const int*)map,
                             (const float*)scale, scale_by_src ? 1 : 0,
                             (const int*)choice, nchoice, (void*)out, rows, d,
                             reinterpret_cast<hipStream_t>(stream));
          hipError_t e = hipGetLastError();
          if (e != hipSuccess) throw std::runtime_error(hipGetErrorString(e));
        });
  m.def("moe_gather2",
        [](int dtype, uintptr_t in, long in_rows, uintptr_t map,
           uintptr_t scale, uintptr_t out, long rows, long d,
           uintptr_t stream) {
          adapcc::moe_gather2(dtype, (const void*)in, in_rows,
                              (const int*)map, (const float*)scale,
                              (void*)out, rows, d,
                              reinterpret_cast<hipStream_t>(stream));
          hipError_t e = hipGetLastError();
          if (e != hipSuccess) throw std::runtime_error(hipGetErrorString(e));
        });
  m.def("moe_rowdot",
        [](int dtype, uintptr_t a, uintptr_t b, long b_rows, uintptr_t map,
           uintptr_t out, long rows, long d, int a_shift, uintptr_t stream) {
          adapcc::moe_rowdot(dtype, (const void*)a, (const void*)b, b_rows,
                             (const int*)map, (float*)out, rows, d, a_shift,
                             reinterpret_cast<hipStream_t>(stream));
          hipError_t e = hipGetLastError();
          if (e != hipSuccess) throw std::runtime_error(hipGetErrorString(e));
        });

  m.def("tr_probe",
        [](uintptr_t out, int kb, int db, uintptr_t stream) {
          adapcc::tr_probe((float*)out, kb, db,
                           reinterpret_cast<hipStream_t>(stream));
          hipError_t e = hipGetLastError();
          if (e != hipSuccess) throw std::runtime_error(hipGetErrorString(e));
        });
  m.def("pack_probe",
        [](uintptr_t out, uintptr_t stream) {
          adapcc::pack_probe((float*)out,
                             reinterpret_cast<hipStream_t>(stream));
          hipError_t e = hipGetLastError();
          if (e != hipSuccess) throw std::runtime_error(hipGetErrorString(e));
        });

  m.def("compute_plan",
        [](const std::vector<std::vector<int>>& parents, int rank,
           long total_elems, int esize, long chunk_bytes,
           const std::vector<int>& active,
           const std::vector<double>& slice_weights) {
          auto shape = adapcc::TreeShape::derive(parents);
          uint64_t mask = 0;
          for (int r : active) mask |= (1ull << r);
          if (active.empty()) mask = (1ull << shape.world) - 1;
          return plan_to_dict(adapcc::build_plan(shape, rank, total_elems,
                                                 esize, chunk_bytes, mask,
                                                 slice_weights));
        },
        py::arg("parents"), py::arg("rank"), py::arg("total_elems"),
        py::arg("esize"), py::arg("chunk_bytes"),
        py::arg("active") = std::vector<int>{},
        py::arg("slice_weights") = std::vector<double>{});

  m.def("compute_primitive_plan",
        [](const std::string& prim, int world, int rank, long elems, int esize,
           long chunk_bytes, int root,
           const std::vector<std::vector<int>>& parents,
           const std::vector<int>& active,
           const std::vector<double>& slice_weights) {
          uint64_t mask = 0;
          for (int r : active) mask |= (1ull << r);
          if (active.empty()) mask = (1ull << world) - 1;
          adapcc::PlanData pd;
          if (prim == "reduce") {
            auto shape = parents.empty() ? adapcc::star_shape(world)
                                         : adapcc::TreeShape::derive(parents);
            pd = adapcc::build_reduce_plan(shape, rank, root, elems, esize,
                                           chunk_bytes, mask, slice_weights);
          } else if (prim == "broadcast") {
            pd = adapcc::build_broadcast_plan(world, rank, root, elems, esize,
                                              chunk_bytes);
          } else if (prim == "allgather") {
            pd = adapcc::build_allgather_plan(world, rank, elems, esize,
                                              chunk_bytes);
          } else if (prim == "reducescatter") {
            pd = adapcc::build_reducescatter_plan(world, rank, elems, esize,
                                                  chunk_bytes, mask);
          } else if (prim == "alltoall") {
            pd = adapcc::build_alltoall_plan(world, rank, elems, esize,
                                             chunk_bytes);
          } else {
            throw std::runtime_error("unknown primitive " + prim);
          }
          return plan_to_dict(pd);
        },
        py::arg("prim"), py::arg("world"), py::arg("rank"), py::arg("elems"),
        py::arg("esize"), py::arg("chunk_bytes"), py::arg("root") = 0,
        py::arg("parents") = std::vector<std::vector<int>>{},
        py::arg("active") = std::vector<int>{},
        py::arg("slice_weights") = std::vector<double>{});

  py::class_<Engine>(m, "Engine")
      .def(py::init<int, int, int, size_t, double>(), py::arg("rank"),
           py::arg("world"), py::arg("device"), py::arg("cap_bytes"),
           py::arg("timeout_ms"))
      .def("ipc_handle",
           [](Engine& e) { return py::bytes(e.ipc_handle()); })
      .def("connect",
           [](Engine& e, const std::vector<py::bytes>& handles,
              const std::vector<int>& peer_devices) {
             std::vector<std::string> hs;
             hs.reserve(handles.size());
             for (const auto& h : handles) hs.push_back(std::string(h));
             e.connect(hs, peer_devices);
           },
           py::arg("handles"), py::arg("peer_devices") = std::vector<int>{})
      .def("set_strategy", &Engine::set_strategy, py::arg("parents"),
           py::arg("chunk_bytes"),
           py::arg("slice_weights") = std::vector<double>{})
      .def("connect_local", &Engine::connect_local, py::arg("peer_addrs"))
      .def("region_addr", &Engine::region_addr)
      .def("allreduce",
           [](Engine& e, uintptr_t data_ptr, long numel, int dtype, int op,
              const std::vector<int>& active, bool average,
              uintptr_t stream) {
             e.allreduce(reinterpret_cast<void*>(data_ptr), numel, dtype, op,
                         active, average, reinterpret_cast<void*>(stream));
           },
           py::arg("data_ptr"), py::arg("numel"), py::arg("dtype"),
           py::arg("op"), py::arg("active"), py::arg("average"),
           py::arg("stream"))
      .def("reduce",
           [](Engine& e, uintptr_t data_ptr, long numel, int dtype, int op,
              int root, const std::vector<int>& active, uintptr_t stream) {
             e.reduce(reinterpret_cast<void*>(data_ptr), numel, dtype, op,
                      root, active, reinterpret_cast<void*>(stream));
           },
           py::arg("data_ptr"), py::arg("numel"), py::arg("dtype"),
           py::arg("op"), py::arg("root"), py::arg("active"),
           py::arg("stream"))
      .def("broadcast",
           [](Engine& e, uintptr_t data_ptr, long numel, int dtype, int root,
              uintptr_t stream) {
             e.broadcast(reinterpret_cast<void*>(data_ptr), numel, dtype, root,
                         reinterpret_cast<void*>(stream));
           },
           py::arg("data_ptr"), py::arg("numel"), py::arg("dtype"),
           py::arg("root"), py::arg("stream"))
      .def("all_gather",
           [](Engine& e, uintptr_t in_ptr, uintptr_t out_ptr, long in_elems,
              int dtype, uintptr_t stream) {
             e.all_gather(reinterpret_cast<const void*>(in_ptr),
                          reinterpret_cast<void*>(out_ptr), in_elems, dtype,
                          reinterpret_cast<void*>(stream));
           },
           py::arg("in_ptr"), py::arg("out_ptr"), py::arg("in_elems"),
           py::arg("dtype"), py::arg("stream"))
      .def("all_to_all",
           [](Engine& e, uintptr_t in_ptr, uintptr_t out_ptr, long per_rank,
              int dtype, uintptr_t stream) {
             e.all_to_all(reinterpret_cast<const void*>(in_ptr),
                          reinterpret_cast<void*>(out_ptr), per_rank, dtype,
                          reinterpret_cast<void*>(stream));
           },
           py::arg("in_ptr"), py::arg("out_ptr"), py::arg("per_rank_elems"),
           py::arg("dtype"), py::arg("stream"))
      .def("reduce_scatter",
           [](Engine& e, uintptr_t in_ptr, uintptr_t out_ptr, long out_elems,
              int dtype, int op, const std::vector<int>& active, bool average,
              uintptr_t stream) {
             e.reduce_scatter(reinterpret_cast<const void*>(in_ptr),
                              reinterpret_cast<void*>(out_ptr), out_elems,
                              dtype, op, active, average,
                              reinterpret_cast<void*>(stream));
           },
           py::arg("in_ptr"), py::arg("out_ptr"), py::arg("out_elems"),
           py::arg("dtype"), py::arg("op"), py::arg("active"),
           py::arg("average"), py::arg("stream"))
      .def("synchronize", &Engine::synchronize,
           py::call_guard<py::gil_scoped_release>())
      .def("query_error", &Engine::query_error)
      .def("dump_inbox", [](Engine& e) { return py::bytes(e.dump_inbox()); })
      .def_property_readonly("rank", &Engine::rank)
      .def_property_readonly("world", &Engine::world)
      .def_property_readonly("capacity", &Engine::capacity)
      .def_property_readonly("num_trees", &Engine::num_trees);

  m.attr("DTYPE_F32") = (int)adapcc::Dtype::F32;
  m.attr("DTYPE_F16") = (int)adapcc::Dtype::F16;
  m.attr("DTYPE_BF16") = (int)adapcc::Dtype::BF16;
  m.attr("OP_SUM") = (int)adapcc::RedOp::Sum;
  m.attr("OP_AVG") = (int)adapcc::RedOp::Avg;
  m.attr("OP_MAX") = (int)adapcc::RedOp::Max;
  m.attr("OP_MIN") = (int)adapcc::RedOp::Min;
  m.attr("MAX_RANKS") = adapcc::kMaxRanks;
  m.attr("MAX_TREES") = adapcc::kMaxTrees;
}
```

adapcc_amd/ops/csrc/ce.hip:

```cpp

#include <hip/hip_runtime.h>
#include <hip/hip_fp16.h>
#include <hip/hip_bf16.h>

#include <cstdint>
#include <stdexcept>
#include <string>

#include "common.h"

namespace adapcc {

namespace {

__device__ __forceinline__ float to_f32(float x) { return x; }
__device__ __forceinline__ float to_f32(__half x) { return __half2float(x); }
__device__ __forceinline__ float to_f32(__hip_bfloat16 x) {
  return __bfloat162float(x);
}

template <typename T>
__device__ __forceinline__ T from_f32(float x);
template <>
__device__ __forceinline__ float from_f32<float>(float x) { return x; }
template <>
__device__ __forceinline__ __half from_f32<__half>(float x) {
  return __float2half(x);
}
template <>
__device__ __forceinline__ __hip_bfloat16 from_f32<__hip_bfloat16>(float x) {
  return __float2bfloat16(x);
}

constexpr float kNegInf = -3.0e38f;

__device__ __forceinline__ void combine(float& m, float& s, float m2,
                                        float s2) {
  const float mn = fmaxf(m, m2);
  s = (m == kNegInf ? 0.f : s * __expf(m - mn)) +
      (m2 == kNegInf ? 0.f : s2 * __expf(m2 - mn));
  m = mn;
}

template <typename T>
struct alignas(16) Pack {
  static constexpr int N = 16 / sizeof(T);
  T v[N];
};

__device__ __forceinline__ void block_reduce_ms(float& m, float& s,
                                                float* lds_m, float* lds_s) {
  for (int off = 32; off > 0; off >>= 1) {
    const float m2 = __shfl_xor(m, off, 64);
    const float s2 = __shfl_xor(s, off, 64);
    combine(m, s, m2, s2);
  }
  const int wave = threadIdx.x >> 6;
  const int lane = threadIdx.x & 63;
  if (lane == 0) {
    lds_m[wave] = m;
    lds_s[wave] = s;
  }
  __syncthreads();
  m = lds_m[0];
  s = lds_s[0];
#pragma unroll
  for (int w = 1; w < 4; ++w) combine(m, s, lds_m[w], lds_s[w]);
}

template <typename T>
__global__ __launch_bounds__(256) void ce_fwd_kernel(
    const T* __restrict__ logits, const long* __restrict__ targets,
    float* __restrict__ loss, float* __restrict__ lse, long cols,
    long ignore_index) {
  constexpr int PK = Pack<T>::N;
  const long row = blockIdx.x;
  const T* x = logits + row * cols;
  const int tid = threadIdx.x;

  const uintptr_t addr = reinterpret_cast<uintptr_t>(x);
  const long head = ((16 - (addr & 15)) & 15) / sizeof(T);
  const long nvec = (cols - head) / PK;
  const long tail_start = head + nvec * PK;

  float m = kNegInf, s = 0.f;
  if (tid < head) {
    const float xv = to_f32(x[tid]);
    m = xv;
    s = 1.f;
  }
  const Pack<T>* xp = reinterpret_cast<const Pack<T>*>(x + head);
  for (long p = tid; p < nvec; p += 256) {
    const Pack<T> pk = xp[p];
    float xv[PK];
#pragma unroll
    for (int j = 0; j < PK; ++j) xv[j] = to_f32(pk.v[j]);
    float lm = xv[0];
#pragma unroll
    for (int j = 1; j < PK; ++j) lm = fmaxf(lm, xv[j]);
    if (lm > m) {
      s *= __expf(m - lm);
      m = lm;
    }
#pragma unroll
    for (int j = 0; j < PK; ++j) s += __expf(xv[j] - m);
  }
  for (long i = tail_start + tid; i < cols; i += 256) {
    const float xv = to_f32(x[i]);
    if (xv > m) {
      s *= __expf(m - xv);
      m = xv;
    }
    s += __expf(xv - m);
  }

  __shared__ float lds_m[4], lds_s[4];
  block_reduce_ms(m, s, lds_m, lds_s);

  if (tid == 0) {
    const float l = m + __logf(s);
    lse[row] = l;
    const long t = targets[row];
    loss[row] =
        (t == ignore_index) ? 0.f : (l - to_f32(x[t]));
  }
}

template <typename T>
__global__ __launch_bounds__(256) void ce_bwd_kernel(
    const T* __restrict__ logits, const long* __restrict__ targets,
    const float* __restrict__ lse, const float* __restrict__ gscale_ptr,
    T* __restrict__ dlogits, long cols, long ignore_index) {
  constexpr int PK = Pack<T>::N;
  const long row = blockIdx.x;
  const T* x = logits + row * cols;
  T* dx = dlogits + row * cols;
  const int tid = threadIdx.x;

  const long t = targets[row];
  const float gscale = (t == ignore_index) ? 0.f : *gscale_ptr;
  const float l = lse[row];

  const uintptr_t addr = reinterpret_cast<uintptr_t>(x);
  const long head = ((16 - (addr & 15)) & 15) / sizeof(T);
  const long nvec = (cols - head) / PK;
  const long tail_start = head + nvec * PK;

  if (tid < head) {
    const float p = __expf(to_f32(x[tid]) - l);
    dx[tid] = from_f32<T>(gscale * (p - (tid == t ? 1.f : 0.f)));
  }
  const Pack<T>* xp = reinterpret_cast<const Pack<T>*>(x + head);
  Pack<T>* dxp = reinterpret_cast<Pack<T>*>(dx + head);
  for (long p = tid; p < nvec; p += 256) {
    const Pack<T> pk = xp[p];
    Pack<T> o;
    const long base = head + p * PK;
#pragma unroll
    for (int j = 0; j < PK; ++j) {
      const float sm = __expf(to_f32(pk.v[j]) - l);
      o.v[j] = from_f32<T>(gscale * (sm - (base + j == t ? 1.f : 0.f)));
    }
    dxp[p] = o;
  }
  for (long i = tail_start + tid; i < cols; i += 256) {
    const float sm = __expf(to_f32(x[i]) - l);
    dx[i] = from_f32<T>(gscale * (sm - (i == t ? 1.f : 0.f)));
  }
}

}

void ce_forward(int dtype, const void* logits, const void* targets,
                float* loss, float* lse, long rows, long cols,
                long ignore_index, hipStream_t stream) {
  const dim3 block(256);
  const dim3 grid((unsigned)rows);
  switch ((Dtype)dtype) {
    case Dtype::F32:
      hipLaunchKernelGGL((ce_fwd_kernel<float>), grid, block, 0, stream,
                         (const float*)logits, (const long*)targets, loss,
                         lse, cols, ignore_index);
      return;
    case Dtype::F16:
      hipLaunchKernelGGL((ce_fwd_kernel<__half>), grid, block, 0, stream,
                         (const __half*)logits, (const long*)targets, loss,
                         lse, cols, ignore_index);
      return;
    case Dtype::BF16:
      hipLaunchKernelGGL((ce_fwd_kernel<__hip_bfloat16>), grid, block, 0,
                         stream, (const __hip_bfloat16*)logits,
                         (const long*)targets, loss, lse, cols, ignore_index);
      return;
  }
  throw std::runtime_error("ce_forward: bad dtype " + std::to_string(dtype));
}

void ce_backward(int dtype, const void* logits, const void* targets,
                 const float* lse, const float* gscale, void* dlogits,
                 long rows, long cols, long ignore_index,
                 hipStream_t stream) {
  const dim3 block(256);
  const dim3 grid((unsigned)rows);
  switch ((Dtype)dtype) {
    case Dtype::F32:
      hipLaunchKernelGGL((ce_bwd_kernel<float>), grid, block, 0, stream,
                         (const float*)logits, (const long*)targets, lse,
                         gscale, (float*)dlogits, cols, ignore_index);
      return;
    case Dtype::F16:
      hipLaunchKernelGGL((ce_bwd_kernel<__half>), grid, block, 0, stream,
                         (const __half*)logits, (const long*)targets, lse,
                         gscale, (__half*)dlogits, cols, ignore_index);
      return;
    case Dtype::BF16:
      hipLaunchKernelGGL((ce_bwd_kernel<__hip_bfloat16>), grid, block, 0,
                         stream, (const __hip_bfloat16*)logits,
                         (const long*)targets, lse, gscale,
                         (__hip_bfloat16*)dlogits, cols, ignore_index);
      return;
  }
  throw std::runtime_error("ce_backward: bad dtype " + std::to_string(dtype));
}

}
```

adapcc_amd/ops/csrc/gelu.hip:

```cpp

#include <hip/hip_runtime.h>
#include <hip/hip_fp16.h>
#include <hip/hip_bf16.h>

#include <cstdint>
#include <stdexcept>
#include <string>

#include "common.h"

namespace adapcc {

namespace {

constexpr float kA = 0.7978845608028654f;
constexpr float kB = 0.044715f;
constexpr float k2Log2e = 2.885390081777927f;

__device__ __forceinline__ float tanh_fast(float z) {
  const float e = __builtin_amdgcn_exp2f(z * k2Log2e);
  return 1.f - 2.f / (e + 1.f);
}

__device__ __forceinline__ float gelu_fwd1(float x) {
  const float u = kA * __builtin_fmaf(kB * x * x, x, x);
  return 0.5f * x * (1.f + tanh_fast(u));
}

__device__ __forceinline__ float gelu_bwd1(float x, float g) {
  const float x2 = x * x;
  const float u = kA * __builtin_fmaf(kB * x2, x, x);
  const float t = tanh_fast(u);
  const float sech2 = 1.f - t * t;
  const float du = kA * __builtin_fmaf(3.f * kB, x2, 1.f);
  return g * (0.5f * (1.f + t) + 0.5f * x * sech2 * du);
}

template <typename T>
struct alignas(16) Pk {
  static constexpr int N = 16 / sizeof(T);
  T v[N];
};

__device__ __forceinline__ float to_f(float x) { return x; }
__device__ __forceinline__ float to_f(__half x) { return __half2float(x); }
__device__ __forceinline__ float to_f(__hip_bfloat16 x) {
  return __bfloat162float(x);
}
template <typename T>
__device__ __forceinline__ T from_f(float x);
template <>
__device__ __forceinline__ float from_f<float>(float x) { return x; }
template <>
__device__ __forceinline__ __half from_f<__half>(float x) {
  return __float2half(x);
}
template <>
__device__ __forceinline__ __hip_bfloat16 from_f<__hip_bfloat16>(float x) {
  return __float2bfloat16(x);
}

template <typename T>
__global__ __launch_bounds__(256) void gelu_fwd_kernel(
    const T* __restrict__ x, T* __restrict__ y, long n) {
  constexpr int PK = Pk<T>::N;
  const long nvec = n / PK;
  const Pk<T>* xv = reinterpret_cast<const Pk<T>*>(x);
  Pk<T>* yv = reinterpret_cast<Pk<T>*>(y);
  for (long i = blockIdx.x * blockDim.x + threadIdx.x; i < nvec;
       i += (long)gridDim.x * blockDim.x) {
    Pk<T> a = xv[i], o;
#pragma unroll
    for (int k = 0; k < PK; ++k) o.v[k] = from_f<T>(gelu_fwd1(to_f(a.v[k])));
    yv[i] = o;
  }
  for (long i = nvec * PK + blockIdx.x * blockDim.x + threadIdx.x; i < n;
       i += (long)gridDim.x * blockDim.x)
    y[i] = from_f<T>(gelu_fwd1(to_f(x[i])));
}

template <typename T>
__global__ __launch_bounds__(256) void gelu_bwd_kernel(
    const T* __restrict__ x, const T* __restrict__ dy, T* __restrict__ dx,
    long n) {
  constexpr int PK = Pk<T>::N;
  const long nvec = n / PK;
  const Pk<T>* xv = reinterpret_cast<const Pk<T>*>(x);
  const Pk<T>* gv = reinterpret_cast<const Pk<T>*>(dy);
  Pk<T>* dv = reinterpret_cast<Pk<T>*>(dx);
  for (long i = blockIdx.x * blockDim.x + threadIdx.x; i < nvec;
       i += (long)gridDim.x * blockDim.x) {
    Pk<T> a = xv[i], g = gv[i], o;
#pragma unroll
    for (int k = 0; k < PK; ++k)
      o.v[k] = from_f<T>(gelu_bwd1(to_f(a.v[k]), to_f(g.v[k])));
    dv[i] = o;
  }
  for (long i = nvec * PK + blockIdx.x * blockDim.x + threadIdx.x; i < n;
       i += (long)gridDim.x * blockDim.x)
    dx[i] = from_f<T>(gelu_bwd1(to_f(x[i]), to_f(dy[i])));
}

}

static dim3 ew_grid(long n) {
  long blocks = (n / 8 + 255) / 256;
  if (blocks > 2048) blocks = 2048;
  if (blocks < 1) blocks = 1;
  return dim3((unsigned)blocks);
}

void gelu_forward(int dtype, const void* x, void* y, long n,
                  hipStream_t stream) {
  switch ((Dtype)dtype) {
    case Dtype::F32:
      hipLaunchKernelGGL((gelu_fwd_kernel<float>), ew_grid(n), dim3(256), 0,
                         stream, (const float*)x, (float*)y, n);
      return;
    case Dtype::F16:
      hipLaunchKernelGGL((gelu_fwd_kernel<__half>), ew_grid(n), dim3(256), 0,
                         stream, (const __half*)x, (__half*)y, n);
      return;
    case Dtype::BF16:
      hipLaunchKernelGGL((gelu_fwd_kernel<__hip_bfloat16>), ew_grid(n),
                         dim3(256), 0, stream, (const __hip_bfloat16*)x,
                         (__hip_bfloat16*)y, n);
      return;
  }
  throw std::runtime_error("gelu_forward: bad dtype");
}

void gelu_backward(int dtype, const void* x, const void* dy, void* dx, long n,
                   hipStream_t stream) {
  switch ((Dtype)dtype) {
    case Dtype::F32:
      hipLaunchKernelGGL((gelu_bwd_kernel<float>), ew_grid(n), dim3(256), 0,
                         stream, (const float*)x, (const float*)dy,
                         (float*)dx, n);
      return;
    case Dtype::F16:
      hipLaunchKernelGGL((gelu_bwd_kernel<__half>), ew_grid(n), dim3(256), 0,
                         stream, (const __half*)x, (const __half*)dy,
                         (__half*)dx, n);
      return;
    case Dtype::BF16:
      hipLaunchKernelGGL((gelu_bwd_kernel<__hip_bfloat16>), ew_grid(n),
                         dim3(256), 0, stream, (const __hip_bfloat16*)x,
                         (const __hip_bfloat16*)dy, (__hip_bfloat16*)dx, n);
      return;
  }
  throw std::runtime_error("gelu_backward: bad dtype");
}

}
```

adapcc_amd/ops/csrc/lnorm.hip:

```cpp

#include <hip/hip_runtime.h>
#include <hip/hip_fp16.h>
#include <hip/hip_bf16.h>

#include "attn_drop.h"
#include "common.h"

#include <stdexcept>
#include <string>

namespace adapcc {

#define DEV_INLINE __device__ __forceinline__

unsigned fa_drop_threshold(double p);

namespace {

template <typename T> struct LnIo;
template <> struct LnIo<float> {
  using Vec = float4;
  static constexpr int kPerVec = 4;
  DEV_INLINE static void unpack(const Vec& v, float* o) {
    o[0] = v.x; o[1] = v.y; o[2] = v.z; o[3] = v.w;
  }
  DEV_INLINE static Vec pack(const float* i) {
    return make_float4(i[0], i[1], i[2], i[3]);
  }
};
template <> struct LnIo<__hip_bfloat16> {
  struct Vec { uint4 raw; };
  static constexpr int kPerVec = 8;
  DEV_INLINE static void unpack(const Vec& v, float* o) {
    const unsigned* w = reinterpret_cast<const unsigned*>(&v.raw);
#pragma unroll
    for (int i = 0; i < 4; ++i) {
      __hip_bfloat162 h = *reinterpret_cast<const __hip_bfloat162*>(&w[i]);
      o[2 * i] = __bfloat162float(h.x);
      o[2 * i + 1] = __bfloat162float(h.y);
    }
  }
  DEV_INLINE static Vec pack(const float* i) {
    Vec v; unsigned* w = reinterpret_cast<unsigned*>(&v.raw);
#pragma unroll
    for (int k = 0; k < 4; ++k) {
      __hip_bfloat162 h{__float2bfloat16(i[2 * k]),
                        __float2bfloat16(i[2 * k + 1])};
      w[k] = *reinterpret_cast<const unsigned*>(&h);
    }
    return v;
  }
};
template <> struct LnIo<__half> {
  struct Vec { uint4 raw; };
  static constexpr int kPerVec = 8;
  DEV_INLINE static void unpack(const Vec& v, float* o) {
    const unsigned* w = reinterpret_cast<const unsigned*>(&v.raw);
#pragma unroll
    for (int i = 0; i < 4; ++i) {
      __half2 h = *reinterpret_cast<const __half2*>(&w[i]);
      o[2 * i] = __half2float(__low2half(h));
      o[2 * i + 1] = __half2float(__high2half(h));
    }
  }
  DEV_INLINE static Vec pack(const float* i) {
    Vec v; unsigned* w = reinterpret_cast<unsigned*>(&v.raw);
#pragma unroll
    for (int k = 0; k < 4; ++k) {
      __half2 h = __floats2half2_rn(i[2 * k], i[2 * k + 1]);
      w[k] = *reinterpret_cast<const unsigned*>(&h);
    }
    return v;
  }
};

DEV_INLINE float wave_sum(float v) {
#pragma unroll
  for (int off = 32; off > 0; off >>= 1) v += __shfl_xor(v, off, 64);
  return v;
}

}

template <typename T, int COLS>
struct RowShape {
  using IO = LnIo<T>;
  static constexpr int PV = IO::kPerVec;
  static_assert(COLS % PV == 0, "COLS must be vector-divisible");
  static constexpr int kVecs = COLS / PV;
  static constexpr int kChunks = (kVecs + 63) / 64;
  static constexpr int kElems = kChunks * PV;
};

struct LnDrop {
  const long* seed;
  unsigned site;
  unsigned thr;
  float scale;
};

DEV_INLINE float ln_scaled_add(float r, float h, float scale) {
#pragma clang fp contract(off)
  return r + h * scale;
}

template <typename T, int COLS, bool kAdd, bool kDrop>
__global__ void __launch_bounds__(256) ln_fwd_kernel(
    const T* __restrict__ x, const T* __restrict__ w, const T* __restrict__ b,
    T* __restrict__ y, float* __restrict__ mean_out,
    float* __restrict__ rstd_out, long rows, float eps,
    const T* __restrict__ h, T* __restrict__ x_new, LnDrop drop) {
  static_assert(kAdd || !kDrop, "dropout acts on the added h");
  using RS = RowShape<T, COLS>;
  using IO = typename RS::IO;
  using Vec = typename IO::Vec;
  constexpr int PV = RS::PV;
  const int lane = threadIdx.x & 63;
  const int wave = threadIdx.x >> 6;
  const long row = (long)blockIdx.x * 4 + wave;
  if (row >= rows) return;

  uint32_t seed_hi = 0, ra = 0;
  if constexpr (kDrop) {
    const uint64_t sd = (uint64_t)*drop.seed;
    seed_hi = (uint32_t)(sd >> 32);
    ra = drop_q_part((uint32_t)sd, drop.site, (uint32_t)row);
  }

  const T* xr = x + row * COLS;
  float vals[RS::kElems];
  float sum = 0.f;
#pragma unroll
  for (int s = 0; s < RS::kChunks; ++s) {
    const int vi = s * 64 + lane;
    if (vi < RS::kVecs) {
      Vec v = reinterpret_cast<const Vec*>(xr)[vi];
      IO::unpack(v, &vals[s * PV]);
      if constexpr (kAdd) {
        float hv[PV];
        Vec vh = reinterpret_cast<const Vec*>(h + row * COLS)[vi];
        IO::unpack(vh, hv);
#pragma unroll
        for (int k = 0; k < PV; ++k) {
          if constexpr (kDrop) {
            const uint32_t cb =
                drop_k_part(seed_hi, drop.site, (uint32_t)(vi * PV + k));
            if (drop_keep_parts(ra, cb, drop.thr))
              vals[s * PV + k] =
                  ln_scaled_add(vals[s * PV + k], hv[k], drop.scale);
          } else {
            vals[s * PV + k] += hv[k];
          }
        }
        v = IO::pack(&vals[s * PV]);
        reinterpret_cast<Vec*>(x_new + row * COLS)[vi] = v;
        IO::unpack(v, &vals[s * PV]);
      }
#pragma unroll
      for (int k = 0; k < PV; ++k) sum += vals[s * PV + k];
    } else {
#pragma unroll
      for (int k = 0; k < PV; ++k) vals[s * PV + k] = 0.f;
    }
  }
  sum = wave_sum(sum);
  const float mean = sum / COLS;
  float var = 0.f;
#pragma unroll
  for (int s = 0; s < RS::kChunks; ++s) {
    if (s * 64 + lane < RS::kVecs) {
#pragma unroll
      for (int k = 0; k < PV; ++k) {
        const float d = vals[s * PV + k] - mean;
        var += d * d;
      }
    }
  }
  var = wave_sum(var);
  const float rstd = rsqrtf(var / COLS + eps);
  if (lane == 0) {
    mean_out[row] = mean;
    rstd_out[row] = rstd;
  }

  T* yr = y + row * COLS;
#pragma unroll
  for (int s = 0; s < RS::kChunks; ++s) {
    const int vi = s * 64 + lane;
    if (vi < RS::kVecs) {
      float wv[PV], bv[PV], out[PV];
      Vec a = reinterpret_cast<const Vec*>(w)[vi];
      Vec c = reinterpret_cast<const Vec*>(b)[vi];
      IO::unpack(a, wv);
      IO::unpack(c, bv);
#pragma unroll
      for (int k = 0; k < PV; ++k)
        out[k] = (vals[s * PV + k] - mean) * rstd * wv[k] + bv[k];
      reinterpret_cast<Vec*>(yr)[vi] = IO::pack(out);
    }
  }
}

template <typename T, int COLS, bool kAdd, bool kDrop>
__global__ void __launch_bounds__(256) ln_bwd_kernel(
    const T* __restrict__ dy, const T* __restrict__ x,
    const T* __restrict__ w, const float* __restrict__ mean_in,
    const float* __restrict__ rstd_in, T* __restrict__ dx,
    float* __restrict__ ws_gamma, float* __restrict__ ws_beta, long rows,
    const T* __restrict__ dx_in, T* __restrict__ dh, LnDrop drop) {
  using RS = RowShape<T, COLS>;
  using IO = typename RS::IO;
  using Vec = typename IO::Vec;
  constexpr int PV = RS::PV;
  const int lane = threadIdx.x & 63;
  const int wave = threadIdx.x >> 6;
  const long wave_stride = (long)gridDim.x * 4;

  float dg[RS::kElems];
  float db[RS::kElems];
#pragma unroll
  for (int i = 0; i < RS::kElems; ++i) dg[i] = db[i] = 0.f;

  float wv[RS::kElems];
#pragma unroll
  for (int s = 0; s < RS::kChunks; ++s) {
    const int vi = s * 64 + lane;
    if (vi < RS::kVecs) {
      Vec v = reinterpret_cast<const Vec*>(w)[vi];
      IO::unpack(v, &wv[s * PV]);
    }
  }

  uint32_t cb[kDrop ? RS::kElems : 1];
  uint32_t seed_lo = 0;
  if constexpr (kDrop) {
    const uint64_t sd = (uint64_t)*drop.seed;
    seed_lo = (uint32_t)sd;
#pragma unroll
    for (int s = 0; s < RS::kChunks; ++s)
#pragma unroll
      for (int k = 0; k < PV; ++k)
        cb[s * PV + k] =
            drop_k_part((uint32_t)(sd >> 32), drop.site,
                        (uint32_t)((s * 64 + lane) * PV + k));
  }

  for (long row = (long)blockIdx.x * 4 + wave; row < rows; row += wave_stride) {
    const T* dyr = dy + row * COLS;
    const T* xr = x + row * COLS;
    const float mean = mean_in[row];
    const float rstd = rstd_in[row];

    float dyv[RS::kElems], xh[RS::kElems];
    Vec vin[kAdd ? RS::kChunks : 1];
    float s1 = 0.f, s2 = 0.f;
#pragma unroll
    for (int s = 0; s < RS::kChunks; ++s) {
      const int vi = s * 64 + lane;
      if (vi < RS::kVecs) {
        float d[PV], xx[PV];
        Vec vd = reinterpret_cast<const Vec*>(dyr)[vi];
        Vec vx = reinterpret_cast<const Vec*>(xr)[vi];
        if constexpr (kAdd)
          vin[s] = reinterpret_cast<const Vec*>(dx_in + row * COLS)[vi];
        IO::unpack(vd, d);
        IO::unpack(vx, xx);
#pragma unroll
        for (int k = 0; k < PV; ++k) {
          const float xhat = (xx[k] - mean) * rstd;
          const float a = d[k] * wv[s * PV + k];
          dyv[s * PV + k] = d[k];
          xh[s * PV + k] = xhat;
          s1 += a;
          s2 += a * xhat;
        }
      }
    }
    s1 = wave_sum(s1) / COLS;
    s2 = wave_sum(s2) / COLS;

    T* dxr = dx + row * COLS;
    uint32_t ra = 0;
    if constexpr (kDrop) ra = drop_q_part(seed_lo, drop.site, (uint32_t)row);
#pragma unroll
    for (int s = 0; s < RS::kChunks; ++s) {
      const int vi = s * 64 + lane;
      if (vi < RS::kVecs) {
        float out[PV];
#pragma unroll
        for (int k = 0; k < PV; ++k) {
          const float a = dyv[s * PV + k] * wv[s * PV + k];
          out[k] = (a - s1 - xh[s * PV + k] * s2) * rstd;
          dg[s * PV + k] += dyv[s * PV + k] * xh[s * PV + k];
          db[s * PV + k] += dyv[s * PV + k];
        }
        if constexpr (kAdd) {
          float gin[PV];
          IO::unpack(vin[s], gin);
#pragma unroll
          for (int k = 0; k < PV; ++k) out[k] += gin[k];
        }
        reinterpret_cast<Vec*>(dxr)[vi] = IO::pack(out);
        if constexpr (kDrop) {
#pragma unroll
          for (int k = 0; k < PV; ++k)
            out[k] = drop_keep_parts(ra, cb[s * PV + k], drop.thr)
                         ? out[k] * drop.scale
                         : 0.f;
          reinterpret_cast<Vec*>(dh + row * COLS)[vi] = IO::pack(out);
        }
      }
    }
  }

  const long slot = (long)blockIdx.x * 4 + wave;
  float* wg = ws_gamma + slot * COLS;
  float* wb = ws_beta + slot * COLS;
#pragma unroll
  for (int s = 0; s < RS::kChunks; ++s) {
    const int vi = s * 64 + lane;
    if (vi < RS::kVecs) {
#pragma unroll
      for (int q = 0; q < PV / 4; ++q) {
        reinterpret_cast<float4*>(wg + vi * PV)[q] =
            make_float4(dg[s * PV + 4 * q], dg[s * PV + 4 * q + 1],
                        dg[s * PV + 4 * q + 2], dg[s * PV + 4 * q + 3]);
        reinterpret_cast<float4*>(wb + vi * PV)[q] =
            make_float4(db[s * PV + 4 * q], db[s * PV + 4 * q + 1],
                        db[s * PV + 4 * q + 2], db[s * PV + 4 * q + 3]);
      }
    }
  }
}


#define LN_COLS_LIST(X) \
  X(128) X(256) X(384) X(512) X(640) X(768) X(1024) X(1280) X(1536) \
  X(2048) X(3072) X(4096)

bool ln_supported_api(long cols, int dtype) {
  const int pv = dtype_size((Dtype)dtype) == 4 ? 4 : 8;
  if (cols % pv) return false;
#define LN_CHECK(C) if (cols == C) return true;
  LN_COLS_LIST(LN_CHECK)
#undef LN_CHECK
  return false;
}

namespace {

struct LnFwdArgs {
  const void *x, *w, *b;
  void* y;
  float *mean, *rstd;
  long rows, cols;
  float eps;
  const void* h;
  void* x_new;
  LnDrop drop;
};

struct LnBwdArgs {
  const void *dy, *x, *w;
  const float *mean, *rstd;
  void* dx;
  float *ws_gamma, *ws_beta;
  long rows, cols;
  int nblocks;
  const void* dx_in;
  void* dh;
  LnDrop drop;
};

template <typename T, bool kAdd, bool kDrop>
void ln_fwd_dispatch(const LnFwdArgs& a, hipStream_t s) {
  const dim3 block(256);
  const dim3 grid((a.rows + 3) / 4);
#define LN_FWD_CASE(C)                                                      \
  if (a.cols == C) {                                                        \
    hipLaunchKernelGGL((ln_fwd_kernel<T, C, kAdd, kDrop>), grid, block, 0,  \
                       s, (const T*)a.x, (const T*)a.w, (const T*)a.b,      \
                       (T*)a.y, a.mean, a.rstd, a.rows, a.eps,              \
                       (const T*)a.h, (T*)a.x_new, a.drop);                 \
    return;                                                                 \
  }
  LN_COLS_LIST(LN_FWD_CASE)
#undef LN_FWD_CASE
  throw std::runtime_error("ln_forward: unsupported cols=" +
                           std::to_string(a.cols) +
                           " (check ln_supported first)");
}

template <typename T, bool kAdd, bool kDrop>
void ln_bwd_dispatch(const LnBwdArgs& a, hipStream_t s) {
  const dim3 block(256);
#define LN_BWD_CASE(C)                                                      \
  if (a.cols == C) {                                                        \
    hipLaunchKernelGGL((ln_bwd_kernel<T, C, kAdd, kDrop>),                  \
                       dim3(a.nblocks), block, 0, s, (const T*)a.dy,        \
                       (const T*)a.x, (const T*)a.w, a.mean, a.rstd,        \
                       (T*)a.dx, a.ws_gamma, a.ws_beta, a.rows,             \
                       (const T*)a.dx_in, (T*)a.dh, a.drop);                \
    return;                                                                 \
  }
  LN_COLS_LIST(LN_BWD_CASE)
#undef LN_BWD_CASE
  throw std::runtime_error("ln_backward: unsupported cols=" +
                           std::to_string(a.cols) +
                           " (check ln_supported first)");
}

template <typename T>
void ln_fwd_typed(const LnFwdArgs& a, bool drop, hipStream_t s) {
  if (a.h == nullptr)
    ln_fwd_dispatch<T, false, false>(a, s);
  else if (drop)
    ln_fwd_dispatch<T, true, true>(a, s);
  else
    ln_fwd_dispatch<T, true, false>(a, s);
}

template <typename T>
void ln_bwd_typed(const LnBwdArgs& a, bool drop, hipStream_t s) {
  const bool add = a.dx_in != nullptr;
  if (drop && add)
    ln_bwd_dispatch<T, true, true>(a, s);
  else if (drop)
    ln_bwd_dispatch<T, false, true>(a, s);
  else if (add)
    ln_bwd_dispatch<T, true, false>(a, s);
  else
    ln_bwd_dispatch<T, false, false>(a, s);
}

void ln_fwd_any(int dtype, const LnFwdArgs& a, bool drop, hipStream_t s) {
  switch ((Dtype)dtype) {
    case Dtype::F32: ln_fwd_typed<float>(a, drop, s); break;
    case Dtype::BF16: ln_fwd_typed<__hip_bfloat16>(a, drop, s); break;
    case Dtype::F16: ln_fwd_typed<__half>(a, drop, s); break;
  }
}

void ln_bwd_any(int dtype, const LnBwdArgs& a, bool drop, hipStream_t s) {
  switch ((Dtype)dtype) {
    case Dtype::F32: ln_bwd_typed<float>(a, drop, s); break;
    case Dtype::BF16: ln_bwd_typed<__hip_bfloat16>(a, drop, s); break;
    case Dtype::F16: ln_bwd_typed<__half>(a, drop, s); break;
  }
}

LnDrop ln_drop_args(const char* name, long rows, double p, const long* seed,
                    unsigned site) {
  if (rows < 1 || rows >= (1L << 32))
    throw std::runtime_error(std::string(name) + ": need 1 <= rows < 2^32");
  if (!(p >= 0.0 && p < 1.0))
    throw std::runtime_error(std::string(name) + ": need 0 <= dropout_p < 1");
  if (p > 0.0 && seed == nullptr)
    throw std::runtime_error(std::string(name) +
                             ": dropout needs a device seed");
  return LnDrop{seed, site, fa_drop_threshold(p), (float)(1.0 / (1.0 - p))};
}

}

void ln_forward(int dtype, const void* x, const void* w, const void* b,
                void* y, float* mean, float* rstd, long rows, long cols,
                float eps, hipStream_t stream) {
  ln_fwd_any(dtype,
             {x, w, b, y, mean, rstd, rows, cols, eps, nullptr, nullptr, {}},
             false, stream);
}

void ln_backward(int dtype, const void* dy, const void* x, const void* w,
                 const float* mean, const float* rstd, void* dx,
                 float* ws_gamma, float* ws_beta, long rows, long cols,
                 int nblocks, hipStream_t stream) {
  ln_bwd_any(dtype,
             {dy, x, w, mean, rstd, dx, ws_gamma, ws_beta, rows, cols, nblocks,
              nullptr, nullptr, {}},
             false, stream);
}

void ln_dropadd_forward(int dtype, const void* h, const void* res,
                        const void* w, const void* b, void* x_new, void* y,
                        float* mean, float* rstd, long rows, long cols,
                        float eps, double dropout_p, const long* seed,
                        unsigned site, hipStream_t stream) {
  const LnDrop drop =
      ln_drop_args("ln_dropadd_forward", rows, dropout_p, seed, site);
  if (h == nullptr || x_new == nullptr)
    throw std::runtime_error("ln_dropadd_forward: null h or x_new");
  ln_fwd_any(dtype,
             {res, w, b, y, mean, rstd, rows, cols, eps, h, x_new, drop},
             dropout_p > 0.0, stream);
}

void ln_dropadd_backward(int dtype, const void* dy, const void* dx_new,
                         const void* x_new, const void* w, const float* mean,
                         const float* rstd, void* dres, void* dh,
                         float* ws_gamma, float* ws_beta, long rows,
                         long cols, int nblocks, double dropout_p,
                         const long* seed, unsigned site,
                         hipStream_t stream) {
  const LnDrop drop =
      ln_drop_args("ln_dropadd_backward", rows, dropout_p, seed, site);
  if (dropout_p > 0.0 && dh == nullptr)
    throw std::runtime_error("ln_dropadd_backward: dropout needs dh");
  if (nblocks < 1)
    throw std::runtime_error("ln_dropadd_backward: nblocks < 1");
  ln_bwd_any(dtype,
             {dy, x_new, w, mean, rstd, dres, ws_gamma, ws_beta, rows, cols,
              nblocks, dx_new, dh, drop},
             dropout_p > 0.0, stream);
}

}
```

adapcc_amd/ops/fused.py:

```python

from __future__ import annotations

from typing import Optional

import torch
import torch.nn as nn

_CORE = None
_DT = {}


def _core():
    global _CORE
    if _CORE is None:
        try:
            from adapcc_amd import _core as c

            _CORE = c
            _DT.update({torch.float32: c.DTYPE_F32, torch.float16: c.DTYPE_F16,
                        torch.bfloat16: c.DTYPE_BF16})
        except ImportError:
            _CORE = False
    return _CORE


def ln_fusable(cols: int, dtype: torch.dtype) -> bool:
    c = _core()
    if not c or dtype not in _DT:
        return False
    return bool(c.ln_supported(cols, _DT[dtype]))


class _FusedLayerNormFn(torch.autograd.Function):
    @staticmethod
    def forward(ctx, x: torch.Tensor, weight: torch.Tensor,
                bias: torch.Tensor, eps: float) -> torch.Tensor:
        c = _core()
        xc = x.contiguous()
        cols = xc.shape[-1]
        rows = xc.numel() // cols
        y = torch.empty_like(xc)
        mean = torch.empty(rows, dtype=torch.float32, device=xc.device)
        rstd = torch.empty_like(mean)
        stream = torch.cuda.current_stream(xc.device).cuda_stream
        c.ln_fwd(_DT[xc.dtype], xc.data_ptr(), weight.data_ptr(),
                 bias.data_ptr(), y.data_ptr(), mean.data_ptr(),
                 rstd.data_ptr(), rows, cols, eps, stream)
        ctx.save_for_backward(xc, weight, mean, rstd)
        return y

    @staticmethod
    def backward(ctx, dy: torch.Tensor):
        c = _core()
        x, weight, mean, rstd = ctx.saved_tensors
        cols = x.shape[-1]
        rows = x.numel() // cols
        dyc = dy.contiguous()
        dx = torch.empty_like(x)
        nblocks = max(1, min(1024, (rows + 3) // 4))
        nslots = nblocks * 4
        ws = torch.empty(2 * nslots * cols, dtype=torch.float32,
                         device=x.device)
        wsg = ws[: nslots * cols]
        wsb = ws[nslots * cols:]
        stream = torch.cuda.current_stream(x.device).cuda_stream
        c.ln_bwd(_DT[x.dtype], dyc.data_ptr(), x.data_ptr(),
                 weight.data_ptr(), mean.data_ptr(), rstd.data_ptr(),
                 dx.data_ptr(), wsg.data_ptr(), wsb.data_ptr(),
                 rows, cols, nblocks, stream)
        dgamma = wsg.view(nslots, cols).sum(0).to(weight.dtype)
        dbeta = wsb.view(nslots, cols).sum(0).to(weight.dtype)
        return dx, dgamma, dbeta, None


class _FusedCrossEntropyFn(torch.autograd.Function):

    @staticmethod
    def forward(ctx, logits: torch.Tensor, targets: torch.Tensor,
                ignore_index: int) -> torch.Tensor:
        c = _core()
        lc = logits.contiguous()
        rows, cols = lc.shape
        tc = targets.contiguous().to(torch.int64)
        loss = torch.empty(rows, dtype=torch.float32, device=lc.device)
        lse = torch.empty_like(loss)
        stream = torch.cuda.current_stream(lc.device).cuda_stream
        c.ce_fwd(_DT[lc.dtype], lc.data_ptr(), tc.data_ptr(),
                 loss.data_ptr(), lse.data_ptr(), rows, cols, ignore_index,
                 stream)
        n_valid = (tc != ignore_index).sum().to(torch.float32).clamp(min=1)
        ctx.save_for_backward(lc, tc, lse, n_valid)
        ctx.ignore_index = ignore_index
        return loss.sum() / n_valid

    @staticmethod
    def backward(ctx, grad_out: torch.Tensor):
        c = _core()
        logits, targets, lse, n_valid = ctx.saved_tensors
        rows, cols = logits.shape
        gscale = (grad_out.to(torch.float32) / n_valid).reshape(1).contiguous()
        dlogits = torch.empty_like(logits)
        stream = torch.cuda.current_stream(logits.device).cuda_stream
        c.ce_bwd(_DT[logits.dtype], logits.data_ptr(), targets.data_ptr(),
                 lse.data_ptr(), gscale.data_ptr(), dlogits.data_ptr(),
                 rows, cols, ctx.ignore_index, stream)
        return dlogits, None, None


def fused_cross_entropy(logits: torch.Tensor, targets: torch.Tensor,
                        ignore_index: int = -100) -> torch.Tensor:
    if (
        logits.is_cuda
        and logits.dim() == 2
        and logits.shape[0] > 0
        and logits.shape[1] > 0
        and _core()
        and logits.dtype in _DT
        and not torch.is_autocast_enabled()
    ):
        return _FusedCrossEntropyFn.apply(logits, targets, ignore_index)
    return torch.nn.functional.cross_entropy(
        logits.float(), targets, ignore_index=ignore_index)


class _FusedGeluFn(torch.autograd.Function):

    @staticmethod
    def forward(ctx, x: torch.Tensor) -> torch.Tensor:
        c = _core()
        xc = x.contiguous()
        y = torch.empty_like(xc)
        stream = torch.cuda.current_stream(xc.device).cuda_stream
        c.gelu_fwd(_DT[xc.dtype], xc.data_ptr(), y.data_ptr(), xc.numel(),
                   stream)
        ctx.save_for_backward(xc)
        return y

    @staticmethod
    def backward(ctx, dy: torch.Tensor):
        c = _core()
        (x,) = ctx.saved_tensors
        dyc = dy.contiguous()
        dx = torch.empty_like(x)
        stream = torch.cuda.current_stream(x.device).cuda_stream
        c.gelu_bwd(_DT[x.dtype], x.data_ptr(), dyc.data_ptr(), dx.data_ptr(),
                   x.numel(), stream)
        return dx


def fused_gelu(x: torch.Tensor) -> torch.Tensor:
    if x.is_cuda and _core() and x.dtype in _DT \
            and not torch.is_autocast_enabled():
        return _FusedGeluFn.apply(x)
    return torch.nn.functional.gelu(x, approximate="tanh")


class FusedLayerNorm(nn.LayerNorm):

    def forward(self, x: torch.Tensor) -> torch.Tensor:
        if (
            x.is_cuda
            and not torch.is_autocast_enabled()
            and len(self.normalized_shape) == 1
            and self.weight is not None
            and self.bias is not None
            and self.weight.dtype == x.dtype
            and ln_fusable(x.shape[-1], x.dtype)
        ):
            return _FusedLayerNormFn.apply(x, self.weight, self.bias,
                                           self.eps)
        return super().forward(x)


def dropout_add_keep_mask_reference(seed, rows: int, cols: int, p: float,
                                    site: int = 0) -> torch.Tensor:
    from .attention import _M32, _drop_threshold, _fmix

    seed = int(seed) & 0xFFFFFFFFFFFFFFFF
    seed_lo, seed_hi = seed & _M32, seed >> 32
    site = int(site) & _M32
    r = torch.arange(rows, dtype=torch.int64).view(-1, 1)
    c = torch.arange(cols, dtype=torch.int64).view(1, -1)
    a = _fmix((seed_lo + site * 0x9E3779B1 + r * 0x85EBCA77) & _M32)
    b = _fmix(((seed_hi ^ ((site * 0xC2B2AE3D) & _M32))
               + c * 0x27D4EB2F) & _M32)
    x = (a + b) & _M32
    x = (x * 0x2C1B3C6D) & _M32
    x = x ^ (x >> 15)
    x = (x * 0x297A2D39) & _M32
    x = x ^ (x >> 15)
    return x >= _drop_threshold(p)


def _dropadd_fusable(h: torch.Tensor, residual: torch.Tensor,
                     weight: torch.Tensor, bias: torch.Tensor) -> bool:
    if not h.is_cuda or torch.is_autocast_enabled():
        return False
    if weight is None or bias is None or h.dim() < 1:
        return False
    if not (h.dtype == residual.dtype == weight.dtype == bias.dtype):
        return False
    if not (h.device == residual.device == weight.device == bias.device):
        return False
    cols = h.shape[-1]
    if weight.shape != (cols,) or bias.shape != (cols,) or cols == 0:
        return False
    if not 1 <= h.numel() // cols < 2 ** 32:
        return False
    return ln_fusable(cols, h.dtype)


def _launch_dropadd_fwd(h, residual, weight, bias, x_new, y, mean, rstd,
                        eps, dropout_p, seed, site):
    cols = h.shape[-1]
    stream = torch.cuda.current_stream(h.device).cuda_stream
    _core().ln_dropadd_fwd(
        _DT[h.dtype], h.data_ptr(), residual.data_ptr(), weight.data_ptr(),
        bias.data_ptr(), x_new.data_ptr(), y.data_ptr(), mean.data_ptr(),
        rstd.data_ptr(), h.numel() // cols, cols, eps, stream, dropout_p,
        seed.data_ptr() if dropout_p > 0.0 else 0, site)


def _launch_dropadd_bwd(dy, dx_new, x_new, weight, mean, rstd, dres, dh,
                        wsg, wsb, nblocks, dropout_p, seed, site):
    cols = x_new.shape[-1]
    stream = torch.cuda.current_stream(x_new.device).cuda_stream
    _core().ln_dropadd_bwd(
        _DT[x_new.dtype], dy.data_ptr(),
        dx_new.data_ptr() if dx_new is not None else 0, x_new.data_ptr(),
        weight.data_ptr(), mean.data_ptr(), rstd.data_ptr(), dres.data_ptr(),
        dh.data_ptr() if dh is not None else 0, wsg.data_ptr(),
        wsb.data_ptr(), x_new.numel() // cols, cols, nblocks, stream,
        dropout_p, seed.data_ptr() if dropout_p > 0.0 else 0, site)


class _DropoutAddLayerNormFn(torch.autograd.Function):

    @staticmethod
    def forward(ctx, h, residual, weight, bias, eps, dropout_p, seed, site):
        hc, rc = h.contiguous(), residual.contiguous()
        cols = rc.shape[-1]
        rows = rc.numel() // cols
        x_new = torch.empty_like(rc)
        y = torch.empty_like(rc)
        mean = torch.empty(rows, dtype=torch.float32, device=rc.device)
        rstd = torch.empty_like(mean)
        _launch_dropadd_fwd(hc, rc, weight, bias, x_new, y, mean, rstd, eps,
                            dropout_p, seed, site)
        ctx.dropout_p, ctx.site = dropout_p, site
        if dropout_p > 0.0:
            ctx.save_for_backward(x_new, weight, mean, rstd, seed)
        else:
            ctx.save_for_backward(x_new, weight, mean, rstd)
        ctx.set_materialize_grads(False)
        return x_new, y

    @staticmethod
    def backward(ctx, dx_new, dy):
        x_new, weight, mean, rstd, *seed = ctx.saved_tensors
        if dx_new is None and dy is None:
            return (None,) * 8
        cols = x_new.shape[-1]
        rows = x_new.numel() // cols
        dyc = dy.contiguous() if dy is not None else torch.zeros_like(x_new)
        dxc = dx_new.contiguous() if dx_new is not None else None
        dres = torch.empty_like(x_new)
        dh = torch.empty_like(x_new) if ctx.dropout_p > 0.0 else None
        nblocks = max(1, min(1024, (rows + 3) // 4))
        nslots = nblocks * 4
        ws = torch.empty(2 * nslots * cols, dtype=torch.float32,
                         device=x_new.device)
        wsg = ws[: nslots * cols]
        wsb = ws[nslots * cols:]
        _launch_dropadd_bwd(dyc, dxc, x_new, weight, mean, rstd, dres, dh,
                            wsg, wsb, nblocks, ctx.dropout_p,
                            seed[0] if seed else None, ctx.site)
        dgamma = wsg.view(nslots, cols).sum(0).to(weight.dtype)
        dbeta = wsb.view(nslots, cols).sum(0).to(weight.dtype)
        return (dh if dh is not None else dres, dres, dgamma, dbeta,
                None, None, None, None)


def _dropout_add_layer_norm_composed(h, residual, weight, bias, eps,
                                     dropout_p, dropout_seed, site):
    from .attention import _seed_tensor

    cols = h.shape[-1]
    if dropout_p > 0.0:
        seed = _seed_tensor(dropout_seed, h.device)
        keep = dropout_add_keep_mask_reference(
            seed, h.numel() // max(cols, 1), cols, dropout_p, site)
        keep = keep.view(h.shape).to(h.device)
        rf = residual.float()
        x_new = torch.where(keep, rf + h.float() * (1.0 / (1.0 - dropout_p)),
                            rf).to(torch.result_type(h, residual))
    else:
        x_new = residual + h
    y = torch.nn.functional.layer_norm(x_new, (cols,), weight, bias, eps)
    return x_new, y


def fused_dropout_add_layer_norm(h: torch.Tensor, residual: torch.Tensor,
                                 weight: torch.Tensor, bias: torch.Tensor,
                                 eps: float = 1e-5, dropout_p: float = 0.0,
                                 dropout_seed: Optional[torch.Tensor] = None,
                                 site: int = 0):
    if not 0.0 <= dropout_p < 1.0:
        raise ValueError("fused_dropout_add_layer_norm: need 0 <= dropout_p "
                         "< 1")
    if not 0 <= site < 2 ** 32:
        raise ValueError("fused_dropout_add_layer_norm: site is a uint32")
    if h.shape != residual.shape:
        raise ValueError("fused_dropout_add_layer_norm: h and residual "
                         "differ in shape")
    if _dropadd_fusable(h, residual, weight, bias):
        from .attention import _seed_tensor

        seed = (_seed_tensor(dropout_seed, h.device) if dropout_p > 0.0
                else None)
        return _DropoutAddLayerNormFn.apply(h, residual, weight, bias, eps,
                                            dropout_p, seed, site)
    return _dropout_add_layer_norm_composed(h, residual, weight, bias, eps,
                                            dropout_p, dropout_seed, site)
```

Before: 774,400 tokens/s.

## Fuse CE gradient into forward, GELU bias-grad, and colsum fold kernels

```diff
diff --git a/adapcc_amd/models/gpt2.py b/adapcc_amd/models/gpt2.py
--- a/adapcc_amd/models/gpt2.py
+++ b/adapcc_amd/models/gpt2.py
@@ -75,8 +75,12 @@
         self.c_proj = nn.Linear(4 * cfg.n_embd, cfg.n_embd)
 
     def forward(self, x: torch.Tensor) -> torch.Tensor:
-        from ..ops.fused import fused_gelu
+        from ..ops.fused import fused_gelu, gelu_bias_grad_fusable
 
+        w, b = self.c_fc.weight, self.c_fc.bias
+        rows = x.numel() // max(x.shape[-1], 1)
+        if gelu_bias_grad_fusable(x.device, x.dtype, rows, w.shape[0], b):
+            return self.c_proj(fused_gelu(F.linear(x, w, b.detach()), bias=b))
         return self.c_proj(fused_gelu(self.c_fc(x)))
 
 
diff --git a/adapcc_amd/ops/build.py b/adapcc_amd/ops/build.py
--- a/adapcc_amd/ops/build.py
+++ b/adapcc_amd/ops/build.py
@@ -10,9 +10,10 @@
 PKG_DIR = os.path.dirname(os.path.dirname(os.path.abspath(__file__)))
 CSRC = os.path.join(PKG_DIR, "ops", "csrc")
 SOURCES = ["kernels.hip", "engine.hip", "plan.cpp", "lnorm.hip", "ce.hip",
-           "attn.hip", "attn_probe.hip", "gelu.hip", "moe.hip",
+           "attn.hip", "attn_probe.hip", "gelu.hip", "moe.hip", "colsum.hip",
            "bindings.hip"]
-HEADERS = ["common.h", "engine.h", "plan.h", "attn_frag.h", "attn_drop.h"]
+HEADERS = ["common.h", "engine.h", "plan.h", "attn_frag.h", "attn_drop.h",
+           "ln_cols.h"]
 OUT_SO = os.path.join(PKG_DIR, "_core.so")
 STAMP = os.path.join(PKG_DIR, "ops", ".build_stamp")
 
diff --git a/adapcc_amd/ops/csrc/attn.hip b/adapcc_amd/ops/csrc/attn.hip
--- a/adapcc_amd/ops/csrc/attn.hip
+++ b/adapcc_amd/ops/csrc/attn.hip
@@ -727,7 +727,7 @@
 
   const int srow = threadIdx.x >> 3;
   const int scol = (threadIdx.x & 7) * 8;
-  const int t0 = kCausal ? (kVarlen ? kt * (kQT / 64) : kt) : 0;
+  const int t0 = kCausal ? kt * (kQT / 64) : 0;
   const int n64 = (S + 63) / 64;
 
   [[maybe_unused]] unsigned dkb = 0, seed_lo = 0;
diff --git a/adapcc_amd/ops/csrc/bindings.hip b/adapcc_amd/ops/csrc/bindings.hip
--- a/adapcc_amd/ops/csrc/bindings.hip
+++ b/adapcc_amd/ops/csrc/bindings.hip
@@ -84,9 +84,18 @@
 void ce_forward(int dtype, const void* logits, const void* targets,
                 float* loss, float* lse, long rows, long cols,
                 long ignore_index, hipStream_t stream);
+long ce_fused_max_cols(int dtype);
+void ce_forward_grad(int dtype, const void* logits, const void* targets,
+                     const float* g0, float* loss, float* lse, void* dlogits,
+                     long rows, long cols, long ignore_index,
+                     hipStream_t stream);
 void ce_backward(int dtype, const void* logits, const void* targets,
-                 const float* lse, const float* gscale, void* dlogits,
-                 long rows, long cols, long ignore_index, hipStream_t stream);
+                 const float* lse, const float* gscale, const float* upstream,
+                 void* dlogits, long rows, long cols, long ignore_index,
+                 hipStream_t stream);
+void colsum_fold(int out_dtype, const float* a0, const float* a1,
+                 const float* a2, void* o0, void* o1, void* o2, long nslots,
+                 long cols, hipStream_t stream);
 void fa_forward(const void* q, const void* k, const void* v, void* o,
                 float* lse, int B, int H, int S, const long* strides,
                 float scale, hipStream_t stream, bool causal,
@@ -119,6 +128,10 @@
                   hipStream_t stream);
 void gelu_backward(int dtype, const void* x, const void* dy, void* dx, long n,
                    hipStream_t stream);
+bool gelu_bias_supported(long cols, int dtype);
+void gelu_backward_bias(int dtype, const void* x, const void* dy, void* dx,
+                        float* ws, long rows, long cols, int nblocks,
+                        hipStream_t stream);
 void moe_route(int dtype, const void* logits, float* gate_p, int* expert,
                int* slot, int* src, int* counts, int* offs, int* totals,
                long ntok, long E, long cap, hipStream_t stream);
@@ -254,12 +267,36 @@
         });
   m.def("ce_bwd",
         [](int dtype, uintptr_t logits, uintptr_t targets, uintptr_t lse,
-           uintptr_t gscale, uintptr_t dlogits, long rows, long cols,
-           long ignore_index, uintptr_t stream) {
+           uintptr_t gscale, uintptr_t upstream, uintptr_t dlogits, long rows,
+           long cols, long ignore_index, uintptr_t stream) {
           adapcc::ce_backward(dtype, (const void*)logits,
                               (const void*)targets, (const float*)lse,
-                              (const float*)gscale, (void*)dlogits, rows,
-                              cols, ignore_index,
+                              (const float*)gscale, (const float*)upstream,
+                              (void*)dlogits, rows, cols, ignore_index,
+                              reinterpret_cast<hipStream_t>(stream));
+          hipError_t e = hipGetLastError();
+          if (e != hipSuccess) throw std::runtime_error(hipGetErrorString(e));
+        });
+  m.def("ce_fused_max_cols", &adapcc::ce_fused_max_cols, py::arg("dtype"));
+  m.def("ce_fwd_grad",
+        [](int dtype, uintptr_t logits, uintptr_t targets, uintptr_t g0,
+           uintptr_t loss, uintptr_t lse, uintptr_t dlogits, long rows,
+           long cols, long ignore_index, uintptr_t stream) {
+          adapcc::ce_forward_grad(dtype, (const void*)logits,
+                                  (const void*)targets, (const float*)g0,
+                                  (float*)loss, (float*)lse, (void*)dlogits,
+                                  rows, cols, ignore_index,
+                                  reinterpret_cast<hipStream_t>(stream));
+          hipError_t e = hipGetLastError();
+          if (e != hipSuccess) throw std::runtime_error(hipGetErrorString(e));
+        });
+  m.def("colsum_fold",
+        [](int out_dtype, uintptr_t a0, uintptr_t a1, uintptr_t a2,
+           uintptr_t o0, uintptr_t o1, uintptr_t o2, long nslots, long cols,
+           uintptr_t stream) {
+          adapcc::colsum_fold(out_dtype, (const float*)a0, (const float*)a1,
+                              (const float*)a2, (void*)o0, (void*)o1,
+                              (void*)o2, nslots, cols,
                               reinterpret_cast<hipStream_t>(stream));
           hipError_t e = hipGetLastError();
           if (e != hipSuccess) throw std::runtime_error(hipGetErrorString(e));
@@ -401,6 +438,19 @@
           adapcc::gelu_backward(dtype, (const void*)x, (const void*)dy,
                                 (void*)dx, n,
                                 reinterpret_cast<hipStream_t>(stream));
+          hipError_t e = hipGetLastError();
+          if (e != hipSuccess) throw std::runtime_error(hipGetErrorString(e));
+        });
+
+  m.def("gelu_bias_supported", &adapcc::gelu_bias_supported, py::arg("cols"),
+        py::arg("dtype"));
+  m.def("gelu_bwd_bias",
+        [](int dtype, uintptr_t x, uintptr_t dy, uintptr_t dx, uintptr_t ws,
+           long rows, long cols, int nblocks, uintptr_t stream) {
+          adapcc::gelu_backward_bias(dtype, (const void*)x, (const void*)dy,
+                                     (void*)dx, (float*)ws, rows, cols,
+                                     nblocks,
+                                     reinterpret_cast<hipStream_t>(stream));
           hipError_t e = hipGetLastError();
           if (e != hipSuccess) throw std::runtime_error(hipGetErrorString(e));
         });
diff --git a/adapcc_amd/ops/csrc/ce.hip b/adapcc_amd/ops/csrc/ce.hip
--- a/adapcc_amd/ops/csrc/ce.hip
+++ b/adapcc_amd/ops/csrc/ce.hip
@@ -67,6 +67,111 @@
 #pragma unroll
   for (int w = 1; w < 4; ++w) combine(m, s, lds_m[w], lds_s[w]);
 }
+
+struct RowSplit {
+  long head, nvec, tail_start;
+};
+
+template <typename T>
+__device__ __forceinline__ RowSplit row_split(const T* x, long cols) {
+  constexpr int PK = Pack<T>::N;
+  const uintptr_t addr = reinterpret_cast<uintptr_t>(x);
+  long head = ((16 - (addr & 15)) & 15) / sizeof(T);
+  if (head > cols) head = cols;
+  const long nvec = (cols - head) / PK;
+  return {head, nvec, head + nvec * PK};
+}
+
+template <int PK>
+__device__ __forceinline__ void accum_vals(float& m, float& s,
+                                           const float (&xv)[PK]) {
+  float lm = xv[0];
+#pragma unroll
+  for (int j = 1; j < PK; ++j) lm = fmaxf(lm, xv[j]);
+  if (lm > m) {
+    s *= __expf(m - lm);
+    m = lm;
+  }
+#pragma unroll
+  for (int j = 0; j < PK; ++j) s += __expf(xv[j] - m);
+}
+
+__device__ __forceinline__ void accum_one(float& m, float& s, float xv) {
+  if (xv > m) {
+    s *= __expf(m - xv);
+    m = xv;
+  }
+  s += __expf(xv - m);
+}
+
+__device__ __forceinline__ float grad_val(float x, float l, float gscale,
+                                          bool is_target) {
+  const float sm = __expf(x - l);
+  return gscale * (sm - (is_target ? 1.f : 0.f));
+}
+
+template <typename T>
+__device__ __forceinline__ T grad_elem(T x, float l, float gscale,
+                                       bool is_target) {
+  return from_f32<T>(grad_val(to_f32(x), l, gscale, is_target));
+}
+
+template <typename T>
+struct Words;
+template <>
+struct Words<float> {
+  __device__ __forceinline__ static void unpack(const uint4& w, float* o) {
+    o[0] = __uint_as_float(w.x);
+    o[1] = __uint_as_float(w.y);
+    o[2] = __uint_as_float(w.z);
+    o[3] = __uint_as_float(w.w);
+  }
+  __device__ __forceinline__ static uint4 pack(const float* i) {
+    return make_uint4(__float_as_uint(i[0]), __float_as_uint(i[1]),
+                      __float_as_uint(i[2]), __float_as_uint(i[3]));
+  }
+};
+template <>
+struct Words<__hip_bfloat16> {
+  __device__ __forceinline__ static void unpack(const uint4& w, float* o) {
+    const unsigned d[4] = {w.x, w.y, w.z, w.w};
+#pragma unroll
+    for (int i = 0; i < 4; ++i) {
+      o[2 * i] = __uint_as_float(d[i] << 16);
+      o[2 * i + 1] = __uint_as_float(d[i] & 0xffff0000u);
+    }
+  }
+  __device__ __forceinline__ static unsigned bits(float x) {
+    return __bfloat16_as_ushort(__float2bfloat16(x));
+  }
+  __device__ __forceinline__ static uint4 pack(const float* i) {
+    return make_uint4(bits(i[0]) | (bits(i[1]) << 16),
+                      bits(i[2]) | (bits(i[3]) << 16),
+                      bits(i[4]) | (bits(i[5]) << 16),
+                      bits(i[6]) | (bits(i[7]) << 16));
+  }
+};
+template <>
+struct Words<__half> {
+  __device__ __forceinline__ static void unpack(const uint4& w, float* o) {
+    const unsigned d[4] = {w.x, w.y, w.z, w.w};
+#pragma unroll
+    for (int i = 0; i < 4; ++i) {
+      o[2 * i] = __half2float(__ushort_as_half((unsigned short)d[i]));
+      o[2 * i + 1] =
+          __half2float(__ushort_as_half((unsigned short)(d[i] >> 16)));
+    }
+  }
+  __device__ __forceinline__ static unsigned bits(float x) {
+    return __half_as_ushort(__float2half(x));
+  }
+  __device__ __forceinline__ static uint4 pack(const float* i) {
+    return make_uint4(bits(i[0]) | (bits(i[1]) << 16),
+                      bits(i[2]) | (bits(i[3]) << 16),
+                      bits(i[4]) | (bits(i[5]) << 16),
+                      bits(i[6]) | (bits(i[7]) << 16));
+  }
+};
 
 template <typename T>
 __global__ __launch_bounds__(256) void ce_fwd_kernel(
@@ -78,41 +183,24 @@
   const T* x = logits + row * cols;
   const int tid = threadIdx.x;
 
-  const uintptr_t addr = reinterpret_cast<uintptr_t>(x);
-  const long head = ((16 - (addr & 15)) & 15) / sizeof(T);
-  const long nvec = (cols - head) / PK;
-  const long tail_start = head + nvec * PK;
+  const RowSplit sp = row_split<T>(x, cols);
 
   float m = kNegInf, s = 0.f;
-  if (tid < head) {
+  if (tid < sp.head) {
     const float xv = to_f32(x[tid]);
     m = xv;
     s = 1.f;
   }
-  const Pack<T>* xp = reinterpret_cast<const Pack<T>*>(x + head);
-  for (long p = tid; p < nvec; p += 256) {
+  const Pack<T>* xp = reinterpret_cast<const Pack<T>*>(x + sp.head);
+  for (long p = tid; p < sp.nvec; p += 256) {
     const Pack<T> pk = xp[p];
     float xv[PK];
 #pragma unroll
     for (int j = 0; j < PK; ++j) xv[j] = to_f32(pk.v[j]);
-    float lm = xv[0];
-#pragma unroll
-    for (int j = 1; j < PK; ++j) lm = fmaxf(lm, xv[j]);
-    if (lm > m) {
-      s *= __expf(m - lm);
-      m = lm;
-    }
-#pragma unroll
-    for (int j = 0; j < PK; ++j) s += __expf(xv[j] - m);
-  }
-  for (long i = tail_start + tid; i < cols; i += 256) {
-    const float xv = to_f32(x[i]);
-    if (xv > m) {
-      s *= __expf(m - xv);
-      m = xv;
-    }
-    s += __expf(xv - m);
-  }
+    accum_vals<PK>(m, s, xv);
+  }
+  for (long i = sp.tail_start + tid; i < cols; i += 256)
+    accum_one(m, s, to_f32(x[i]));
 
   __shared__ float lds_m[4], lds_s[4];
   block_reduce_ms(m, s, lds_m, lds_s);
@@ -121,8 +209,7 @@
     const float l = m + __logf(s);
     lse[row] = l;
     const long t = targets[row];
-    loss[row] =
-        (t == ignore_index) ? 0.f : (l - to_f32(x[t]));
+    loss[row] = (t == ignore_index) ? 0.f : (l - to_f32(x[t]));
   }
 }
 
@@ -130,43 +217,153 @@
 __global__ __launch_bounds__(256) void ce_bwd_kernel(
     const T* __restrict__ logits, const long* __restrict__ targets,
     const float* __restrict__ lse, const float* __restrict__ gscale_ptr,
-    T* __restrict__ dlogits, long cols, long ignore_index) {
+    const float* __restrict__ upstream, T* __restrict__ dlogits, long rows,
+    long cols, long ignore_index) {
+  constexpr int PK = Pack<T>::N;
+  if (upstream != nullptr && *upstream == 1.0f) return;
+  const int tid = threadIdx.x;
+
+  for (long row = blockIdx.x; row < rows; row += gridDim.x) {
+    const T* x = logits + row * cols;
+    T* dx = dlogits + row * cols;
+
+    const long t = targets[row];
+    const float gscale = (t == ignore_index) ? 0.f : *gscale_ptr;
+    const float l = lse[row];
+
+    const RowSplit sp = row_split<T>(x, cols);
+
+    if (tid < sp.head) dx[tid] = grad_elem(x[tid], l, gscale, tid == t);
+    const Pack<T>* xp = reinterpret_cast<const Pack<T>*>(x + sp.head);
+    Pack<T>* dxp = reinterpret_cast<Pack<T>*>(dx + sp.head);
+    for (long p = tid; p < sp.nvec; p += 256) {
+      const Pack<T> pk = xp[p];
+      Pack<T> o;
+      const long base = sp.head + p * PK;
+#pragma unroll
+      for (int j = 0; j < PK; ++j)
+        o.v[j] = grad_elem(pk.v[j], l, gscale, base + j == t);
+      dxp[p] = o;
+    }
+    for (long i = sp.tail_start + tid; i < cols; i += 256)
+      dx[i] = grad_elem(x[i], l, gscale, i == t);
+  }
+}
+
+template <typename T, int NV>
+__global__ __launch_bounds__(256, 3) void ce_fwd_grad_kernel(
+    const T* __restrict__ logits, const long* __restrict__ targets,
+    const float* __restrict__ g0_ptr, float* __restrict__ loss,
+    float* __restrict__ lse, T* __restrict__ dlogits, long cols,
+    long ignore_index) {
   constexpr int PK = Pack<T>::N;
   const long row = blockIdx.x;
   const T* x = logits + row * cols;
   T* dx = dlogits + row * cols;
   const int tid = threadIdx.x;
 
+  const RowSplit sp = row_split<T>(x, cols);
+  const bool has_head = tid < sp.head;
+  const long ti = sp.tail_start + tid;
+  const bool has_tail = ti < cols;
+
+  const uint4* xp =
+      sp.nvec > 0 ? reinterpret_cast<const uint4*>(x + sp.head)
+                  : reinterpret_cast<const uint4*>(
+                        reinterpret_cast<const char*>(x) -
+                        (reinterpret_cast<uintptr_t>(x) & 15));
+  uint4 r[NV];
+#pragma unroll
+  for (int k = 0; k < NV; ++k) {
+    const long p = tid + k * 256;
+    r[k] = xp[p < sp.nvec ? p : 0];
+  }
+  const T xh = x[has_head ? tid : 0];
+  const T xt = x[has_tail ? ti : 0];
+
+  float m = kNegInf, s = 0.f;
+  if (has_head) {
+    m = to_f32(xh);
+    s = 1.f;
+  }
+#pragma unroll
+  for (int k = 0; k < NV; ++k) {
+    asm volatile(""
+                 : "+v"(r[k].x), "+v"(r[k].y), "+v"(r[k].z), "+v"(r[k].w),
+                   "+v"(m));
+    if (tid + k * 256 < sp.nvec) {
+      float xv[PK];
+      Words<T>::unpack(r[k], xv);
+      accum_vals<PK>(m, s, xv);
+    }
+  }
+  if (has_tail) accum_one(m, s, to_f32(xt));
+
+  __shared__ float lds_m[4], lds_s[4];
+  block_reduce_ms(m, s, lds_m, lds_s);
+
+  const float l = m + __logf(s);
   const long t = targets[row];
-  const float gscale = (t == ignore_index) ? 0.f : *gscale_ptr;
-  const float l = lse[row];
-
-  const uintptr_t addr = reinterpret_cast<uintptr_t>(x);
-  const long head = ((16 - (addr & 15)) & 15) / sizeof(T);
-  const long nvec = (cols - head) / PK;
-  const long tail_start = head + nvec * PK;
-
-  if (tid < head) {
-    const float p = __expf(to_f32(x[tid]) - l);
-    dx[tid] = from_f32<T>(gscale * (p - (tid == t ? 1.f : 0.f)));
-  }
-  const Pack<T>* xp = reinterpret_cast<const Pack<T>*>(x + head);
-  Pack<T>* dxp = reinterpret_cast<Pack<T>*>(dx + head);
-  for (long p = tid; p < nvec; p += 256) {
-    const Pack<T> pk = xp[p];
-    Pack<T> o;
-    const long base = head + p * PK;
-#pragma unroll
-    for (int j = 0; j < PK; ++j) {
-      const float sm = __expf(to_f32(pk.v[j]) - l);
-      o.v[j] = from_f32<T>(gscale * (sm - (base + j == t ? 1.f : 0.f)));
+  if (tid == 0) {
+    lse[row] = l;
+    loss[row] = (t == ignore_index) ? 0.f : (l - to_f32(x[t]));
+  }
+
+  const float gscale = (t == ignore_index) ? 0.f : *g0_ptr;
+  if (has_head) dx[tid] = grad_elem(xh, l, gscale, tid == t);
+  uint4* dxp = reinterpret_cast<uint4*>(dx + sp.head);
+#pragma unroll
+  for (int k = 0; k < NV; ++k) {
+    const long p = tid + k * 256;
+    if (p < sp.nvec) {
+      asm volatile(""
+                   : "+v"(r[k].x), "+v"(r[k].y), "+v"(r[k].z), "+v"(r[k].w)
+                   :
+                   : "memory");
+      float xv[PK];
+      Words<T>::unpack(r[k], xv);
+      const long base = sp.head + p * PK;
+#pragma unroll
+      for (int j = 0; j < PK; ++j)
+        xv[j] = grad_val(xv[j], l, gscale, base + j == t);
+      (dxp + k * 256)[tid] = Words<T>::pack(xv);
     }
-    dxp[p] = o;
-  }
-  for (long i = tail_start + tid; i < cols; i += 256) {
-    const float sm = __expf(to_f32(x[i]) - l);
-    dx[i] = from_f32<T>(gscale * (sm - (i == t ? 1.f : 0.f)));
-  }
+  }
+  if (has_tail) dx[ti] = grad_elem(xt, l, gscale, ti == t);
+}
+
+constexpr int kCeMaxVecs = 25;
+
+template <typename T>
+void ce_fwd_grad_launch(const void* logits, const void* targets,
+                        const float* g0, float* loss, float* lse,
+                        void* dlogits, long rows, long cols,
+                        long ignore_index, hipStream_t stream) {
+  const dim3 block(256);
+  const dim3 grid((unsigned)rows);
+  const long vecs = (cols / Pack<T>::N + 255) / 256;
+#define CE_FG_LAUNCH(NV)                                                     \
+  hipLaunchKernelGGL((ce_fwd_grad_kernel<T, NV>), grid, block, 0, stream,    \
+                     (const T*)logits, (const long*)targets, g0, loss, lse,  \
+                     (T*)dlogits, cols, ignore_index)
+  if (vecs <= 4)
+    CE_FG_LAUNCH(4);
+  else if (vecs <= 13)
+    CE_FG_LAUNCH(13);
+  else
+    CE_FG_LAUNCH(kCeMaxVecs);
+#undef CE_FG_LAUNCH
+}
+
+template <typename T>
+void ce_bwd_launch(const void* logits, const void* targets, const float* lse,
+                   const float* gscale, const float* upstream, void* dlogits,
+                   long rows, long cols, long ignore_index,
+                   hipStream_t stream) {
+  const long nb = (upstream != nullptr && rows > 2048) ? 2048 : rows;
+  hipLaunchKernelGGL((ce_bwd_kernel<T>), dim3((unsigned)nb), dim3(256), 0,
+                     stream, (const T*)logits, (const long*)targets, lse,
+                     gscale, upstream, (T*)dlogits, rows, cols, ignore_index);
 }
 
 }
@@ -196,28 +393,57 @@
   throw std::runtime_error("ce_forward: bad dtype " + std::to_string(dtype));
 }
 
-void ce_backward(int dtype, const void* logits, const void* targets,
-                 const float* lse, const float* gscale, void* dlogits,
-                 long rows, long cols, long ignore_index,
-                 hipStream_t stream) {
-  const dim3 block(256);
-  const dim3 grid((unsigned)rows);
+long ce_fused_max_cols(int dtype) {
+  switch ((Dtype)dtype) {
+    case Dtype::F32: return (long)kCeMaxVecs * 256 * Pack<float>::N;
+    case Dtype::F16:
+    case Dtype::BF16: return (long)kCeMaxVecs * 256 * Pack<__half>::N;
+  }
+  return 0;
+}
+
+void ce_forward_grad(int dtype, const void* logits, const void* targets,
+                     const float* g0, float* loss, float* lse, void* dlogits,
+                     long rows, long cols, long ignore_index,
+                     hipStream_t stream) {
+  if (cols < 1 || cols > ce_fused_max_cols(dtype))
+    throw std::runtime_error("ce_forward_grad: cols=" + std::to_string(cols) +
+                             " outside [1, ce_fused_max_cols]");
   switch ((Dtype)dtype) {
     case Dtype::F32:
-      hipLaunchKernelGGL((ce_bwd_kernel<float>), grid, block, 0, stream,
-                         (const float*)logits, (const long*)targets, lse,
-                         gscale, (float*)dlogits, cols, ignore_index);
+      ce_fwd_grad_launch<float>(logits, targets, g0, loss, lse, dlogits, rows,
+                                cols, ignore_index, stream);
       return;
     case Dtype::F16:
-      hipLaunchKernelGGL((ce_bwd_kernel<__half>), grid, block, 0, stream,
-                         (const __half*)logits, (const long*)targets, lse,
-                         gscale, (__half*)dlogits, cols, ignore_index);
+      ce_fwd_grad_launch<__half>(logits, targets, g0, loss, lse, dlogits,
+                                 rows, cols, ignore_index, stream);
       return;
     case Dtype::BF16:
-      hipLaunchKernelGGL((ce_bwd_kernel<__hip_bfloat16>), grid, block, 0,
-                         stream, (const __hip_bfloat16*)logits,
-                         (const long*)targets, lse, gscale,
-                         (__hip_bfloat16*)dlogits, cols, ignore_index);
+      ce_fwd_grad_launch<__hip_bfloat16>(logits, targets, g0, loss, lse,
+                                         dlogits, rows, cols, ignore_index,
+                                         stream);
+      return;
+  }
+  throw std::runtime_error("ce_forward_grad: bad dtype " +
+                           std::to_string(dtype));
+}
+
+void ce_backward(int dtype, const void* logits, const void* targets,
+                 const float* lse, const float* gscale, const float* upstream,
+                 void* dlogits, long rows, long cols, long ignore_index,
+                 hipStream_t stream) {
+  switch ((Dtype)dtype) {
+    case Dtype::F32:
+      ce_bwd_launch<float>(logits, targets, lse, gscale, upstream, dlogits,
+                           rows, cols, ignore_index, stream);
+      return;
+    case Dtype::F16:
+      ce_bwd_launch<__half>(logits, targets, lse, gscale, upstream, dlogits,
+                            rows, cols, ignore_index, stream);
+      return;
+    case Dtype::BF16:
+      ce_bwd_launch<__hip_bfloat16>(logits, targets, lse, gscale, upstream,
+                                    dlogits, rows, cols, ignore_index, stream);
       return;
   }
   throw std::runtime_error("ce_backward: bad dtype " + std::to_string(dtype));
diff --git a/adapcc_amd/ops/csrc/colsum.hip b/adapcc_amd/ops/csrc/colsum.hip
--- /dev/null
+++ b/adapcc_amd/ops/csrc/colsum.hip
@@ -0,0 +1,123 @@
+
+#include <hip/hip_runtime.h>
+#include <hip/hip_fp16.h>
+#include <hip/hip_bf16.h>
+
+#include <stdexcept>
+#include <string>
+
+#include "common.h"
+
+namespace adapcc {
+
+namespace {
+
+constexpr int kFoldCols = 32;
+constexpr int kFoldLanes = 8;
+constexpr int kFoldGroups = 128;
+
+struct FoldArgs {
+  const float* in[3];
+  void* out[3];
+};
+
+__device__ __forceinline__ void fold_store(float* o, float v) { *o = v; }
+__device__ __forceinline__ void fold_store(__half* o, float v) {
+  *o = __float2half(v);
+}
+__device__ __forceinline__ void fold_store(__hip_bfloat16* o, float v) {
+  *o = __float2bfloat16(v);
+}
+
+template <typename T>
+__global__ __launch_bounds__(1024) void colsum_fold_kernel(FoldArgs a,
+                                                           long nslots,
+                                                           long cols) {
+  const float* __restrict__ src = a.in[blockIdx.y];
+  T* __restrict__ dst = static_cast<T*>(a.out[blockIdx.y]);
+  const int cl = threadIdx.x % kFoldLanes;
+  const int sg = threadIdx.x / kFoldLanes;
+  const long c = (long)blockIdx.x * kFoldCols + cl * 4;
+  const bool live = c < cols;
+
+  float4 acc = make_float4(0.f, 0.f, 0.f, 0.f);
+  if (live) {
+#pragma unroll 4
+    for (long s = sg; s < nslots; s += kFoldGroups) {
+      const float4 v = *reinterpret_cast<const float4*>(src + s * cols + c);
+      acc.x += v.x;
+      acc.y += v.y;
+      acc.z += v.z;
+      acc.w += v.w;
+    }
+  }
+
+  __shared__ float4 part[kFoldGroups][kFoldLanes];
+  part[sg][cl] = acc;
+  __syncthreads();
+#pragma unroll
+  for (int h = kFoldGroups / 2; h > 0; h >>= 1) {
+    if (sg < h) {
+      const float4 o = part[sg + h][cl];
+      float4 m = part[sg][cl];
+      m.x += o.x;
+      m.y += o.y;
+      m.z += o.z;
+      m.w += o.w;
+      part[sg][cl] = m;
+    }
+    __syncthreads();
+  }
+  if (sg == 0 && live) {
+    const float4 r = part[0][cl];
+    fold_store(dst + c, r.x);
+    fold_store(dst + c + 1, r.y);
+    fold_store(dst + c + 2, r.z);
+    fold_store(dst + c + 3, r.w);
+  }
+}
+
+}
+
+void colsum_fold(int out_dtype, const float* a0, const float* a1,
+                 const float* a2, void* o0, void* o1, void* o2, long nslots,
+                 long cols, hipStream_t stream) {
+  if (nslots < 1 || cols < 4 || cols % 4 != 0)
+    throw std::runtime_error("colsum_fold: need nslots >= 1 and cols a "
+                             "positive multiple of 4, got " +
+                             std::to_string(nslots) + " x " +
+                             std::to_string(cols));
+  const float* in[3] = {a0, a1, a2};
+  void* out[3] = {o0, o1, o2};
+  FoldArgs args = {};
+  unsigned n = 0;
+  for (int i = 0; i < 3; ++i) {
+    if ((in[i] == nullptr) != (out[i] == nullptr))
+      throw std::runtime_error("colsum_fold: array without its output");
+    if (in[i] == nullptr) continue;
+    args.in[n] = in[i];
+    args.out[n] = out[i];
+    ++n;
+  }
+  if (n == 0) throw std::runtime_error("colsum_fold: no array");
+  const dim3 grid((unsigned)((cols + kFoldCols - 1) / kFoldCols), n);
+  const dim3 block(kFoldLanes * kFoldGroups);
+  switch ((Dtype)out_dtype) {
+    case Dtype::F32:
+      hipLaunchKernelGGL((colsum_fold_kernel<float>), grid, block, 0, stream,
+                         args, nslots, cols);
+      return;
+    case Dtype::F16:
+      hipLaunchKernelGGL((colsum_fold_kernel<__half>), grid, block, 0, stream,
+                         args, nslots, cols);
+      return;
+    case Dtype::BF16:
+      hipLaunchKernelGGL((colsum_fold_kernel<__hip_bfloat16>), grid, block, 0,
+                         stream, args, nslots, cols);
+      return;
+  }
+  throw std::runtime_error("colsum_fold: bad dtype " +
+                           std::to_string(out_dtype));
+}
+
+}
diff --git a/adapcc_amd/ops/csrc/gelu.hip b/adapcc_amd/ops/csrc/gelu.hip
--- a/adapcc_amd/ops/csrc/gelu.hip
+++ b/adapcc_amd/ops/csrc/gelu.hip
@@ -6,8 +6,10 @@
 #include <cstdint>
 #include <stdexcept>
 #include <string>
+#include <type_traits>
 
 #include "common.h"
+#include "ln_cols.h"
 
 namespace adapcc {
 
@@ -36,6 +38,16 @@
   return g * (0.5f * (1.f + t) + 0.5f * x * sech2 * du);
 }
 
+__device__ __forceinline__ float gelu_bwd1_pinned(float x, float g) {
+#pragma clang fp contract(off)
+  const float x2 = x * x;
+  const float u = kA * __builtin_fmaf(kB * x2, x, x);
+  const float t = tanh_fast(u);
+  const float sech2 = __builtin_fmaf(-t, t, 1.f);
+  const float du = kA * __builtin_fmaf(3.f * kB, x2, 1.f);
+  return g * __builtin_fmaf(0.5f * x * sech2, du, 0.5f * (1.f + t));
+}
+
 template <typename T>
 struct alignas(16) Pk {
   static constexpr int N = 16 / sizeof(T);
@@ -58,6 +70,14 @@
 template <>
 __device__ __forceinline__ __hip_bfloat16 from_f<__hip_bfloat16>(float x) {
   return __float2bfloat16(x);
+}
+
+template <typename T>
+__device__ __forceinline__ float gelu_bwd_vec1(float x, float g) {
+  if constexpr (std::is_same<T, __hip_bfloat16>::value)
+    return gelu_bwd1_pinned(x, g);
+  else
+    return gelu_bwd1(x, g);
 }
 
 template <typename T>
@@ -93,12 +113,90 @@
     Pk<T> a = xv[i], g = gv[i], o;
 #pragma unroll
     for (int k = 0; k < PK; ++k)
-      o.v[k] = from_f<T>(gelu_bwd1(to_f(a.v[k]), to_f(g.v[k])));
+      o.v[k] = from_f<T>(gelu_bwd_vec1<T>(to_f(a.v[k]), to_f(g.v[k])));
     dv[i] = o;
   }
   for (long i = nvec * PK + blockIdx.x * blockDim.x + threadIdx.x; i < n;
        i += (long)gridDim.x * blockDim.x)
     dx[i] = from_f<T>(gelu_bwd1(to_f(x[i]), to_f(dy[i])));
+}
+
+template <typename T, int COLS>
+__global__ __launch_bounds__(256) void gelu_bwd_bias_kernel(
+    const T* __restrict__ x, const T* __restrict__ dy, T* __restrict__ dx,
+    float* __restrict__ ws, long rows) {
+  constexpr int PK = Pk<T>::N;
+  static_assert(COLS % PK == 0, "COLS must be vector-divisible");
+  constexpr int kVecs = COLS / PK;
+  constexpr int kChunks = (kVecs + 63) / 64;
+  const int lane = threadIdx.x & 63;
+  const int wave = threadIdx.x >> 6;
+  const long wave_stride = (long)gridDim.x * 4;
+
+  float acc[kChunks * PK];
+#pragma unroll
+  for (int i = 0; i < kChunks * PK; ++i) acc[i] = 0.f;
+
+  for (long row = (long)blockIdx.x * 4 + wave; row < rows;
+       row += wave_stride) {
+    const Pk<T>* xv = reinterpret_cast<const Pk<T>*>(x + row * COLS);
+    const Pk<T>* gv = reinterpret_cast<const Pk<T>*>(dy + row * COLS);
+    Pk<T>* dv = reinterpret_cast<Pk<T>*>(dx + row * COLS);
+#pragma unroll
+    for (int s = 0; s < kChunks; ++s) {
+      const int vi = s * 64 + lane;
+      if (vi < kVecs) {
+        const Pk<T> a = xv[vi], g = gv[vi];
+        Pk<T> o;
+#pragma unroll
+        for (int k = 0; k < PK; ++k) {
+          o.v[k] = from_f<T>(gelu_bwd1_pinned(to_f(a.v[k]), to_f(g.v[k])));
+          acc[s * PK + k] += to_f(o.v[k]);
+        }
+        dv[vi] = o;
+      }
+    }
+  }
+
+  __shared__ __attribute__((aligned(16))) float red[COLS];
+#pragma unroll
+  for (int w = 0; w < 4; ++w) {
+    if (wave == w) {
+#pragma unroll
+      for (int s = 0; s < kChunks; ++s) {
+        const int vi = s * 64 + lane;
+        if (vi < kVecs) {
+#pragma unroll
+          for (int k = 0; k < PK; ++k)
+            red[vi * PK + k] =
+                w == 0 ? acc[s * PK + k] : red[vi * PK + k] + acc[s * PK + k];
+        }
+      }
+    }
+    __syncthreads();
+  }
+  float* wr = ws + (long)blockIdx.x * COLS;
+  for (int i = threadIdx.x * 4; i < COLS; i += 1024)
+    *reinterpret_cast<float4*>(wr + i) =
+        *reinterpret_cast<const float4*>(red + i);
+}
+
+template <typename T>
+void gelu_bwd_bias_dispatch(const void* x, const void* dy, void* dx,
+                            float* ws, long rows, long cols, int nblocks,
+                            hipStream_t stream) {
+#define GELU_BIAS_CASE(C)                                                  \
+  if (cols == C) {                                                         \
+    hipLaunchKernelGGL((gelu_bwd_bias_kernel<T, C>), dim3(nblocks),        \
+                       dim3(256), 0, stream, (const T*)x, (const T*)dy,    \
+                       (T*)dx, ws, rows);                                  \
+    return;                                                                \
+  }
+  LN_COLS_LIST(GELU_BIAS_CASE)
+#undef GELU_BIAS_CASE
+  throw std::runtime_error("gelu_backward_bias: unsupported cols=" +
+                           std::to_string(cols) +
+                           " (check gelu_bias_supported first)");
 }
 
 }
@@ -152,4 +250,26 @@
   throw std::runtime_error("gelu_backward: bad dtype");
 }
 
-}
+bool gelu_bias_supported(long cols, int dtype) {
+  if ((Dtype)dtype != Dtype::BF16) return false;
+#define GELU_BIAS_CHECK(C) if (cols == C) return true;
+  LN_COLS_LIST(GELU_BIAS_CHECK)
+#undef GELU_BIAS_CHECK
+  return false;
+}
+
+void gelu_backward_bias(int dtype, const void* x, const void* dy, void* dx,
+                        float* ws, long rows, long cols, int nblocks,
+                        hipStream_t stream) {
+  if (rows < 1 || nblocks < 1 || nblocks > (rows + 3) / 4)
+    throw std::runtime_error("gelu_backward_bias: need rows >= 1 and "
+                             "1 <= nblocks <= ceil(rows / 4)");
+  if ((Dtype)dtype == Dtype::BF16) {
+    gelu_bwd_bias_dispatch<__hip_bfloat16>(x, dy, dx, ws, rows, cols, nblocks,
+                                           stream);
+    return;
+  }
+  throw std::runtime_error("gelu_backward_bias: bf16 only");
+}
+
+}
diff --git a/adapcc_amd/ops/csrc/ln_cols.h b/adapcc_amd/ops/csrc/ln_cols.h
--- /dev/null
+++ b/adapcc_amd/ops/csrc/ln_cols.h
@@ -0,0 +1,5 @@
+#pragma once
+
+#define LN_COLS_LIST(X) \
+  X(128) X(256) X(384) X(512) X(640) X(768) X(1024) X(1280) X(1536) \
+  X(2048) X(3072) X(4096)
diff --git a/adapcc_amd/ops/csrc/lnorm.hip b/adapcc_amd/ops/csrc/lnorm.hip
--- a/adapcc_amd/ops/csrc/lnorm.hip
+++ b/adapcc_amd/ops/csrc/lnorm.hip
@@ -5,6 +5,7 @@
 
 #include "attn_drop.h"
 #include "common.h"
+#include "ln_cols.h"
 
 #include <stdexcept>
 #include <string>
@@ -333,10 +334,6 @@
   }
 }
 
-
-#define LN_COLS_LIST(X) \
-  X(128) X(256) X(384) X(512) X(640) X(768) X(1024) X(1280) X(1536) \
-  X(2048) X(3072) X(4096)
 
 bool ln_supported_api(long cols, int dtype) {
   const int pv = dtype_size((Dtype)dtype) == 4 ? 4 : 8;
diff --git a/adapcc_amd/ops/fused.py b/adapcc_amd/ops/fused.py
--- a/adapcc_amd/ops/fused.py
+++ b/adapcc_amd/ops/fused.py
@@ -8,6 +8,10 @@
 
 _CORE = None
 _DT = {}
+
+FUSE_CE_GRAD = True
+FUSE_GELU_BIAS_GRAD = True
+FUSE_COLSUM_FOLD = True
 
 
 def _core():
@@ -29,6 +33,19 @@
     if not c or dtype not in _DT:
         return False
     return bool(c.ln_supported(cols, _DT[dtype]))
+
+
+def _fold_partials(parts, nslots: int, cols: int, dtype: torch.dtype):
+    if not (FUSE_COLSUM_FOLD and cols % 4 == 0 and dtype in _DT):
+        return [p.view(nslots, cols).sum(0).to(dtype) for p in parts]
+    dev = parts[0].device
+    outs = [torch.empty(cols, dtype=dtype, device=dev) for _ in parts]
+    pad = [0] * (3 - len(parts))
+    _core().colsum_fold(
+        _DT[dtype], *([p.data_ptr() for p in parts] + pad),
+        *([o.data_ptr() for o in outs] + pad), nslots, cols,
+        torch.cuda.current_stream(dev).cuda_stream)
+    return outs
 
 
 class _FusedLayerNormFn(torch.autograd.Function):
@@ -68,8 +85,7 @@
                  weight.data_ptr(), mean.data_ptr(), rstd.data_ptr(),
                  dx.data_ptr(), wsg.data_ptr(), wsb.data_ptr(),
                  rows, cols, nblocks, stream)
-        dgamma = wsg.view(nslots, cols).sum(0).to(weight.dtype)
-        dbeta = wsb.view(nslots, cols).sum(0).to(weight.dtype)
+        dgamma, dbeta = _fold_partials([wsg, wsb], nslots, cols, weight.dtype)
         return dx, dgamma, dbeta, None
 
 
@@ -77,7 +93,7 @@
 
     @staticmethod
     def forward(ctx, logits: torch.Tensor, targets: torch.Tensor,
-                ignore_index: int) -> torch.Tensor:
+                ignore_index: int, want_grad: bool = False) -> torch.Tensor:
         c = _core()
         lc = logits.contiguous()
         rows, cols = lc.shape
@@ -85,26 +101,42 @@
         loss = torch.empty(rows, dtype=torch.float32, device=lc.device)
         lse = torch.empty_like(loss)
         stream = torch.cuda.current_stream(lc.device).cuda_stream
-        c.ce_fwd(_DT[lc.dtype], lc.data_ptr(), tc.data_ptr(),
-                 loss.data_ptr(), lse.data_ptr(), rows, cols, ignore_index,
-                 stream)
         n_valid = (tc != ignore_index).sum().to(torch.float32).clamp(min=1)
-        ctx.save_for_backward(lc, tc, lse, n_valid)
         ctx.ignore_index = ignore_index
+        ctx.fused = bool(FUSE_CE_GRAD and want_grad
+                         and cols <= c.ce_fused_max_cols(_DT[lc.dtype]))
+        if ctx.fused:
+            g0 = (torch.ones_like(n_valid) / n_valid).reshape(1)
+            dlogits = torch.empty_like(lc)
+            c.ce_fwd_grad(_DT[lc.dtype], lc.data_ptr(), tc.data_ptr(),
+                          g0.data_ptr(), loss.data_ptr(), lse.data_ptr(),
+                          dlogits.data_ptr(), rows, cols, ignore_index, stream)
+            ctx.save_for_backward(lc, tc, lse, n_valid, dlogits)
+            ctx.dlogits_fresh = True
+        else:
+            c.ce_fwd(_DT[lc.dtype], lc.data_ptr(), tc.data_ptr(),
+                     loss.data_ptr(), lse.data_ptr(), rows, cols,
+                     ignore_index, stream)
+            ctx.save_for_backward(lc, tc, lse, n_valid)
         return loss.sum() / n_valid
 
     @staticmethod
     def backward(ctx, grad_out: torch.Tensor):
         c = _core()
-        logits, targets, lse, n_valid = ctx.saved_tensors
+        logits, targets, lse, n_valid, *saved = ctx.saved_tensors
         rows, cols = logits.shape
-        gscale = (grad_out.to(torch.float32) / n_valid).reshape(1).contiguous()
-        dlogits = torch.empty_like(logits)
+        up = grad_out.to(torch.float32).reshape(1).contiguous()
+        gscale = up / n_valid
+        if ctx.fused and ctx.dlogits_fresh:
+            ctx.dlogits_fresh = False
+            dlogits, up_ptr = saved[0], up.data_ptr()
+        else:
+            dlogits, up_ptr = torch.empty_like(logits), 0
         stream = torch.cuda.current_stream(logits.device).cuda_stream
         c.ce_bwd(_DT[logits.dtype], logits.data_ptr(), targets.data_ptr(),
-                 lse.data_ptr(), gscale.data_ptr(), dlogits.data_ptr(),
-                 rows, cols, ctx.ignore_index, stream)
-        return dlogits, None, None
+                 lse.data_ptr(), gscale.data_ptr(), up_ptr,
+                 dlogits.data_ptr(), rows, cols, ctx.ignore_index, stream)
+        return dlogits, None, None, None
 
 
 def fused_cross_entropy(logits: torch.Tensor, targets: torch.Tensor,
@@ -118,7 +150,9 @@
         and logits.dtype in _DT
         and not torch.is_autocast_enabled()
     ):
-        return _FusedCrossEntropyFn.apply(logits, targets, ignore_index)
+        return _FusedCrossEntropyFn.apply(
+            logits, targets, ignore_index,
+            torch.is_grad_enabled() and logits.requires_grad)
     return torch.nn.functional.cross_entropy(
         logits.float(), targets, ignore_index=ignore_index)
 
@@ -148,9 +182,64 @@
         return dx
 
 
-def fused_gelu(x: torch.Tensor) -> torch.Tensor:
-    if x.is_cuda and _core() and x.dtype in _DT \
-            and not torch.is_autocast_enabled():
+class _FusedGeluBiasFn(torch.autograd.Function):
+
+    @staticmethod
+    def forward(ctx, x: torch.Tensor, bias: torch.Tensor) -> torch.Tensor:
+        c = _core()
+        xc = x.contiguous()
+        y = torch.empty_like(xc)
+        stream = torch.cuda.current_stream(xc.device).cuda_stream
+        c.gelu_fwd(_DT[xc.dtype], xc.data_ptr(), y.data_ptr(), xc.numel(),
+                   stream)
+        ctx.save_for_backward(xc)
+        ctx.bias_dtype = bias.dtype
+        return y
+
+    @staticmethod
+    def backward(ctx, dy: torch.Tensor):
+        c = _core()
+        (x,) = ctx.saved_tensors
+        cols = x.shape[-1]
+        rows = x.numel() // cols
+        dyc = dy.contiguous()
+        dx = torch.empty_like(x)
+        nblocks = max(1, min(1024, (rows + 3) // 4))
+        ws = torch.empty(nblocks * cols, dtype=torch.float32, device=x.device)
+        stream = torch.cuda.current_stream(x.device).cuda_stream
+        c.gelu_bwd_bias(_DT[x.dtype], x.data_ptr(), dyc.data_ptr(),
+                        dx.data_ptr(), ws.data_ptr(), rows, cols, nblocks,
+                        stream)
+        (dbias,) = _fold_partials([ws], nblocks, cols, ctx.bias_dtype)
+        return dx, dbias
+
+
+def _gelu_kernel_path(device: torch.device, dtype: torch.dtype) -> bool:
+    return bool(device.type == "cuda" and _core() and dtype in _DT
+                and not torch.is_autocast_enabled())
+
+
+def gelu_bias_grad_fusable(device: torch.device, dtype: torch.dtype,
+                           rows: int, cols: int,
+                           bias: Optional[torch.Tensor]) -> bool:
+    if not (FUSE_GELU_BIAS_GRAD and bias is not None and rows >= 1
+            and cols >= 1 and _gelu_kernel_path(device, dtype)):
+        return False
+    if not (torch.is_grad_enabled() and bias.requires_grad):
+        return False
+    if bias.device != device or bias.dtype not in _DT \
+            or bias.shape != (cols,):
+        return False
+    return bool(_core().gelu_bias_supported(cols, _DT[dtype]))
+
+
+def fused_gelu(x: torch.Tensor,
+               bias: Optional[torch.Tensor] = None) -> torch.Tensor:
+    if _gelu_kernel_path(x.device, x.dtype):
+        cols = x.shape[-1] if x.dim() >= 1 else 0
+        if gelu_bias_grad_fusable(x.device, x.dtype,
+                                  x.numel() // max(cols, 1), cols, bias):
+            return _FusedGeluBiasFn.apply(x, bias)
         return _FusedGeluFn.apply(x)
     return torch.nn.functional.gelu(x, approximate="tanh")
 
@@ -275,8 +364,7 @@
         _launch_dropadd_bwd(dyc, dxc, x_new, weight, mean, rstd, dres, dh,
                             wsg, wsb, nblocks, ctx.dropout_p,
                             seed[0] if seed else None, ctx.site)
-        dgamma = wsg.view(nslots, cols).sum(0).to(weight.dtype)
-        dbeta = wsb.view(nslots, cols).sum(0).to(weight.dtype)
+        dgamma, dbeta = _fold_partials([wsg, wsb], nslots, cols, weight.dtype)
         return (dh if dh is not None else dres, dres, dgamma, dbeta,
                 None, None, None, None)
 
```

New measurement: 801,200 tokens/s (median of 6 runs). 1.03x the previous value.
